# f4exb/sdrdaemon

Hardware: AMD Instinct MI355X
Metric: IQ Msamples/s through decim+FEC-encode pipe; bit-exact vs CPU ref (higher is better)
Workload: dtype int32

## Files before the change

sdrdaemon_amd/csrc/decim_body.h:

```cpp
#pragma once
#include "sdrhip_internal.h"

namespace sdrhip {
namespace {

constexpr int NT = 256;
constexpr int P0 = DECIM_PASS;
constexpr int FULL = 512;
constexpr int HE = 32;

typedef short short2_t __attribute__((ext_vector_type(2)));
typedef int int2_t __attribute__((ext_vector_type(2)));
typedef int int4_t __attribute__((ext_vector_type(4)));
typedef unsigned uint4_t __attribute__((ext_vector_type(4)));

constexpr int C64[16] = {-7, 11, -20, 32, -49, 71, -101, 140, -190, 256, -345, 469, -656, 978, -1698, 5201};
__host__ __device__ constexpr int H32(int i) { return i < 16 ? C64[i] : C64[31 - i]; }
__host__ __device__ constexpr unsigned pack_taps(int lo, int hi) { return ((unsigned)lo & 0xffffu) | ((unsigned)hi << 16); }

constexpr int PK0_DW = 16 + 512 + 16;
constexpr int I0_DW = 32 + 1024;
constexpr int SN_DW = 32 + FULL;

template <int NS_, bool PK_> struct Geo {
    static constexpr int NS = NS_;
    static constexpr bool PK = PK_;
    static constexpr int stride(int s) { return s == 0 ? (PK ? PK0_DW : I0_DW) : SN_DW; }
    static constexpr int base(int s) { return s == 0 ? 0 : base(s - 1) + 4 * stride(s - 1); }
    static constexpr int ldsDw = base(NS);
    static constexpr int plane(int s, int parity, int comp) { return base(s) + (parity * 2 + comp) * stride(s); }
};

__device__ __forceinline__ int dot2(unsigned a, unsigned taps, int acc)
{
    return __builtin_amdgcn_sdot2(__builtin_bit_cast(short2_t, a), __builtin_bit_cast(short2_t, taps), acc, false);
}

__device__ __forceinline__ int dot2_link(unsigned a, unsigned taps, int acc) { return dot2(a, taps, acc); }

__device__ __forceinline__ int dot2_init(unsigned a, unsigned taps, int c)
{
    int d;
    asm("v_dot2_i32_i16 %0, %1, %2, %3" : "=v"(d) : "v"(a), "s"(taps), "v"(c));
    return d;
}

__device__ __forceinline__ int mad24(int a, int tap, int acc)
{
    int d;
    asm("v_mad_i32_i24 %0, %1, %2, %3" : "=v"(d) : "v"(a), "s"(tap), "v"(acc));
    return d;
}

struct OutCtx {
    unsigned *out;
    size_t out_pos;
    bool store;
    int norm, trunk;
    int frame_mode, frame_blocks;
    uint64_t frame_sample_base;
};

__device__ __forceinline__ unsigned final_pack(int i, int q, int norm, int trunk)
{
    int a = (int)((unsigned)i << norm) >> trunk;
    int b = (int)((unsigned)q << norm) >> trunk;
    return ((unsigned)a & 0xffffu) | ((unsigned)b << 16);
}

__device__ __forceinline__ void store_one(const OutCtx &oc, size_t k, unsigned v)
{
    if (!oc.frame_mode) {
        oc.out[k] = v;
    } else {
        uint64_t g = oc.frame_sample_base + k;
        uint64_t f = g / 16129u;
        unsigned w = (unsigned)(g - f * 16129u);
        unsigned b = w / 127u, i = w - b * 127u;
        oc.out[((size_t)f * oc.frame_blocks + 1 + b) * 128u + 1 + i] = v;
    }
}

struct NoTaps { static constexpr bool ON = false; };
struct StageTaps {
    static constexpr bool ON = true;
    const DecimTapArgs &t;
    int stream;
    size_t pos[6];
};

template <class G, int S, class TAPS = NoTaps>
__device__ __forceinline__ void run_stage(int *lds, int tid, int valid, int fill_next, int bias, const OutCtx &oc, TAPS *taps = nullptr)
{
    constexpr bool PK = G::PK && S == 0;
    constexpr bool LAST = (S == G::NS - 1);
    constexpr int R = (S == 0) ? 8 : 4;
    const int j = tid >> 1, comp = tid & 1;
    const int k0 = j * R;
    if (k0 >= valid) return;
    const int *pe = lds + G::plane(S, 0, 0) + comp * G::stride(S);
    const int *po = lds + G::plane(S, 1, 0) + comp * G::stride(S);
    int res[R];
    if constexpr (PK) {
        constexpr int WO = (R + 32) / 2, WE = R / 2 + 4;
        unsigned wo[WO], we[WE];
#pragma unroll
        for (int d = 0; d < WO; d += 4) {
            uint4_t v = *reinterpret_cast<const uint4_t *>(po + k0 / 2 + d);
            wo[d] = v.x; wo[d + 1] = v.y; wo[d + 2] = v.z; wo[d + 3] = v.w;
        }
#pragma unroll
        for (int d = 0; d < WE; d += 4) {
            uint4_t v = *reinterpret_cast<const uint4_t *>(pe + k0 / 2 + 8 + d);
            we[d] = v.x; we[d + 1] = v.y; we[d + 2] = v.z; we[d + 3] = v.w;
        }
        const int bias13 = bias << 13;
        int acc[R];
#pragma unroll
        for (int r = 0; r < R; ++r)
            acc[r] = (r & 1) ? dot2_init(we[(r + 1) / 2], pack_taps(8192, 0), bias13) : dot2_init(we[r / 2], pack_taps(0, 8192), bias13);
#pragma unroll
        for (int t = 0; t < 17; ++t) {
#pragma unroll
            for (int r = 0; r < R; ++r) {
                if (r & 1) {
                    if (t < 16) acc[r] = dot2_link(wo[(r + 1) / 2 + t], pack_taps(H32(31 - 2 * t), H32(30 - 2 * t)), acc[r]);
                } else {
                    const unsigned taps = t == 0 ? pack_taps(0, H32(31)) : (t == 16 ? pack_taps(H32(0), 0) : pack_taps(H32(32 - 2 * t), H32(31 - 2 * t)));
                    acc[r] = dot2_link(wo[r / 2 + t], taps, acc[r]);
                }
            }
        }
#pragma unroll
        for (int r = 0; r < R; ++r) res[r] = acc[r] >> 13;
    } else {
        int wo[R + 32], we[R + 4];
#pragma unroll
        for (int x = 0; x < R + 32; x += 4) {
            int4_t v = *reinterpret_cast<const int4_t *>(po + k0 + x);
            wo[x] = v.x; wo[x + 1] = v.y; wo[x + 2] = v.z; wo[x + 3] = v.w;
        }
#pragma unroll
        for (int x = 0; x < R + 4; x += 4) {
            int4_t v = *reinterpret_cast<const int4_t *>(pe + k0 + 16 + x);
            we[x] = v.x; we[x + 1] = v.y; we[x + 2] = v.z; we[x + 3] = v.w;
        }
        int acc[R];
#pragma unroll
        for (int r = 0; r < R; ++r) acc[r] = (int)((unsigned)(we[r + 1] + bias) << 13);
#pragma unroll
        for (int i = 0; i < 16; ++i) {
#pragma unroll
            for (int r = 0; r < R; ++r) acc[r] = mad24(wo[r + 32 - i] + wo[r + 1 + i], C64[i], acc[r]);
        }
#pragma unroll
        for (int r = 0; r < R; ++r) res[r] = acc[r] >> 13;
    }

    if constexpr (LAST) {
        unsigned o[R];
#pragma unroll
        for (int r = 0; r < R; ++r) {
            int other = __builtin_amdgcn_update_dpp(0, res[r], 0xB1 , 0xf, 0xf, true);
            o[r] = final_pack(res[r], other, oc.norm, oc.trunk);
        }
        if (comp != 0 || !oc.store) return;
        const size_t k = oc.out_pos + k0;
        if (!oc.frame_mode && k0 + R <= valid) {
#pragma unroll
            for (int r = 0; r < R; r += 4) *reinterpret_cast<uint4_t *>(oc.out + k + r) = (uint4_t){o[r], o[r + 1], o[r + 2], o[r + 3]};
        } else if (!oc.frame_mode) {
#pragma unroll
            for (int r = 0; r < R; ++r)
                if (k0 + r < valid) oc.out[k + r] = o[r];
        } else {
            const uint64_t g = oc.frame_sample_base + k;
            const uint64_t f = g / 16129u;
            const unsigned w = (unsigned)(g - f * 16129u);
            unsigned b = w / 127u, i = w - b * 127u;
            size_t dw = ((size_t)f * oc.frame_blocks + 1 + b) * 128u + 1 + i;
#pragma unroll
            for (int r = 0; r < R; ++r) {
                if (k0 + r < valid) oc.out[dw] = o[r];
                ++i; ++dw;
                if (i == 127u) {
                    i = 0; ++b; dw += 1;
                    if (b == 127u) { b = 0; dw += ((size_t)oc.frame_blocks - 127u) * 128u; }
                }
            }
        }
    } else {
        int *ne = lds + G::plane(S + 1, 0, 0) + comp * G::stride(S + 1) + HE + fill_next + k0 / 2;
        int *no = lds + G::plane(S + 1, 1, 0) + comp * G::stride(S + 1) + HE + fill_next + k0 / 2;
        if constexpr (R == 8) {
            *reinterpret_cast<int4_t *>(ne) = (int4_t){res[0], res[2], res[4], res[6]};
            *reinterpret_cast<int4_t *>(no) = (int4_t){res[1], res[3], res[5], res[7]};
        } else {
            *reinterpret_cast<int2_t *>(ne) = (int2_t){res[0], res[2]};
            *reinterpret_cast<int2_t *>(no) = (int2_t){res[1], res[3]};
        }
        if constexpr (TAPS::ON) {
            if (oc.store && (taps->t.mask & (2u << S))) {
                const int norm = taps->t.norm[S + 1], trunk = taps->t.trunk[S + 1];
                unsigned o[R];
#pragma unroll
                for (int r = 0; r < R; ++r) {
                    int other = __builtin_amdgcn_update_dpp(0, res[r], 0xB1 , 0xf, 0xf, true);
                    o[r] = final_pack(res[r], other, norm, trunk);
                }
                if (comp == 0) {
                    unsigned *out = reinterpret_cast<unsigned *>(taps->t.out[S + 1]) + (size_t)taps->stream * taps->t.stride[S + 1] + taps->pos[S] + k0;
                    if (k0 + R <= valid) {
#pragma unroll
                        for (int r = 0; r < R; r += 4) *reinterpret_cast<uint4_t *>(out + r) = (uint4_t){o[r], o[r + 1], o[r + 2], o[r + 3]};
                    } else {
#pragma unroll
                        for (int r = 0; r < R; ++r)
                            if (k0 + r < valid) out[r] = o[r];
                    }
                }
            }
        }
    }
}

template <class G, int S> __device__ __forceinline__ void slide(int *lds, int tid, int consumed)
{
    if (tid >= 128) return;
    const int p = tid >> 5, e = tid & 31;
    int *pl = lds + G::base(S) + p * G::stride(S);
    if constexpr (G::PK && S == 0) {
        short *ps = reinterpret_cast<short *>(pl);
        const short v = ps[e + consumed];
        ps[e] = v;
    } else {
        const int v = pl[e + consumed];
        pl[e] = v;
    }
}

template <class G, int S> __device__ __forceinline__ void hist_put(int *lds, int p, int e, int v)
{
    int *pl = lds + G::base(S) + p * G::stride(S);
    if constexpr (G::PK && S == 0) reinterpret_cast<short *>(pl)[e] = (short)v;
    else pl[e] = v;
}
template <class G, int S> __device__ __forceinline__ int hist_get(const int *lds, int p, int e)
{
    const int *pl = lds + G::base(S) + p * G::stride(S);
    if constexpr (G::PK && S == 0) return reinterpret_cast<const short *>(pl)[e];
    else return pl[e];
}

template <class G, int S = 0> __device__ __forceinline__ void state_load(int *lds, int tid, const int32_t *st, bool zero)
{
    if (tid < 128) {
        const int sp = tid >> 5, e = tid & 31;
        const int kp = (sp & 1) * 2 + (sp >> 1);
        hist_put<G, S>(lds, kp, e, zero ? 0 : st[S * 4 * DEC_HIST + sp * DEC_HIST + e]);
    }
    if constexpr (S + 1 < G::NS) state_load<G, S + 1>(lds, tid, st, zero);
}
template <class G, int S = 0> __device__ __forceinline__ void state_store(const int *lds, int tid, int32_t *st)
{
    if (tid < 128) {
        const int sp = tid >> 5, e = tid & 31;
        const int kp = (sp & 1) * 2 + (sp >> 1);
        st[S * 4 * DEC_HIST + sp * DEC_HIST + e] = hist_get<G, S>(lds, kp, e);
    }
    if constexpr (S + 1 < G::NS) state_store<G, S + 1>(lds, tid, st);
}

template <class G, int S, class TAPS = NoTaps>
__device__ __forceinline__ void later_stages(int *lds, int tid, int (&fill)[6], int consumed_prev, bool flush, int bias, OutCtx &oc, TAPS *taps = nullptr)
{
    if constexpr (S < G::NS) {
        slide<G, S - 1>(lds, tid, consumed_prev);
        fill[S] += consumed_prev / 2;
        const int have = fill[S];
        const bool run = have > 0 && (have >= FULL || flush);
        if (run) {
            run_stage<G, S, TAPS>(lds, tid, have, fill[S + 1 < 6 ? S + 1 : 5], bias, oc, taps);
            if (S == G::NS - 1 && oc.store) oc.out_pos += have;
            if constexpr (TAPS::ON && S < G::NS - 1) {
                if (oc.store) taps->pos[S] += have;
            }
            fill[S] = 0;
        }
        __syncthreads();
        if (run) later_stages<G, S + 1, TAPS>(lds, tid, fill, have, flush, bias, oc, taps);
    } else {
        slide<G, G::NS - 1>(lds, tid, consumed_prev);
        __syncthreads();
    }
}

template <int L, int FC, bool PACK16, bool TAB = true, class TAPS = NoTaps>
__device__ __forceinline__ void decim_piece(const DecimArgs &a, int *lds, int stream, size_t seg_start, size_t seg_end, bool from_state,
                                            bool store_state, int meta_id, int meta_n, TAPS *taps = nullptr)
{
    constexpr bool CEN = (FC == 2);
    constexpr int NS = CEN ? L : L - 2;
    constexpr int RAWSH = CEN ? 0 : 2;
    constexpr int PRAW = P0 << RAWSH;
    constexpr int NLD = PRAW / 4 / NT;
    constexpr int WRAW = 64 << L;
    using G = Geo<NS, PACK16>;
    const int tid = threadIdx.x;
    const unsigned *in = reinterpret_cast<const unsigned *>(a.in) + (size_t)stream * a.in_stride;

    const int32_t *stc = a.state_cur + (size_t)stream * DEC_STATE_WORDS;
    state_load<G>(lds, tid, stc, !from_state);

    OutCtx oc;
    oc.norm = a.norm; oc.trunk = a.trunk;
    oc.frame_mode = a.frame_mode; oc.frame_blocks = a.frame_blocks; oc.frame_sample_base = a.frame_sample_base;
    oc.out = reinterpret_cast<unsigned *>(a.out) + (size_t)stream * a.out_stride;
    oc.out_pos = seg_start >> L;
    if constexpr (TAPS::ON) {
        static_assert(CEN, "taps: centred cascades only");
#pragma unroll
        for (int k = 0; k < 6; ++k) taps->pos[k] = seg_start >> (k + 1);
    }

    if (a.frame_mode) {
        unsigned base[6], rate;
        stream_meta_base(a.meta_w, a.meta_rate, TAB ? a.meta_tab : nullptr, stream, base, rate);
        for (int fi = meta_id + tid * meta_n; fi < a.meta_count; fi += NT * meta_n) {
            unsigned w[6];
            frame_meta_words_thread(base, a.meta_idx0, rate, fi, w);
            unsigned *fr = oc.out + (size_t)(a.meta_first + fi) * a.frame_blocks * 128u;
            fr[0] = (a.meta_frame_count0 + (unsigned)fi) & 0xffffu;
#pragma unroll
            for (int k = 0; k < 6; ++k) fr[1 + k] = w[k];
        }
        if (tid < 128) {
            for (int fi = meta_id; fi < a.meta_count; fi += meta_n) {
                unsigned *fr = oc.out + (size_t)(a.meta_first + fi) * a.frame_blocks * 128u;
                const unsigned fidx = (a.meta_frame_count0 + (unsigned)fi) & 0xffffu;
                if (tid >= 7) fr[tid] = 0u;
                if (tid >= 1) fr[(size_t)tid * 128] = fidx | ((unsigned)tid << 16);
            }
        }
    }

    int fill[6] = {0, 0, 0, 0, 0, 0};
    bool warm = !from_state;
    size_t pos = warm ? seg_start - WRAW : 0;
    size_t region_end = warm ? seg_start : seg_end;

    uint4_t ld[NLD];
    auto issue = [&](size_t p, size_t rend) {
        const unsigned *src = in + p;
        const size_t left = rend - p;
        if (left >= (size_t)PRAW) {
#pragma unroll
            for (int n = 0; n < NLD; ++n) ld[n] = SDRHIP_STREAM_LOAD(reinterpret_cast<const uint4_t *>(src + 4 * (tid + n * NT)));
            return;
        }
        const unsigned rem = (unsigned)left;
#pragma unroll
        for (int n = 0; n < NLD; ++n) {
            const unsigned q = (unsigned)(tid + n * NT);
            uint4_t v = (uint4_t){0u, 0u, 0u, 0u};
            if (4 * q + 3 < rem) {
                v = SDRHIP_STREAM_LOAD(reinterpret_cast<const uint4_t *>(src + 4 * q));
            } else if (4 * q < rem) {
                v.x = src[4 * q];
                if (4 * q + 1 < rem) v.y = src[4 * q + 1];
                if (4 * q + 2 < rem) v.z = src[4 * q + 2];
            }
            ld[n] = v;
        }
    };
    issue(pos, region_end);
    __syncthreads();

    while (true) {
        const size_t left = region_end - pos;
        const int cnt_raw = left < (size_t)PRAW ? (int)left : PRAW;
        const int cnt0 = cnt_raw >> RAWSH;
#pragma unroll
        for (int n = 0; n < NLD; ++n) {
            const int q = tid + n * NT;
            const uint4_t v = ld[n];
            if constexpr (CEN && PACK16) {
                lds[G::plane(0, 0, 0) + 16 + q] = (int)__builtin_amdgcn_perm(v.z, v.x, 0x05040100u);
                lds[G::plane(0, 0, 1) + 16 + q] = (int)__builtin_amdgcn_perm(v.z, v.x, 0x07060302u);
                lds[G::plane(0, 1, 0) + 16 + q] = (int)__builtin_amdgcn_perm(v.w, v.y, 0x05040100u);
                lds[G::plane(0, 1, 1) + 16 + q] = (int)__builtin_amdgcn_perm(v.w, v.y, 0x07060302u);
            } else if constexpr (CEN) {
                *reinterpret_cast<int2_t *>(&lds[G::plane(0, 0, 0) + HE + 2 * q]) = (int2_t){(int)(short)(v.x & 0xffff), (int)(short)(v.z & 0xffff)};
                *reinterpret_cast<int2_t *>(&lds[G::plane(0, 0, 1) + HE + 2 * q]) = (int2_t){(int)v.x >> 16, (int)v.z >> 16};
                *reinterpret_cast<int2_t *>(&lds[G::plane(0, 1, 0) + HE + 2 * q]) = (int2_t){(int)(short)(v.y & 0xffff), (int)(short)(v.w & 0xffff)};
                *reinterpret_cast<int2_t *>(&lds[G::plane(0, 1, 1) + HE + 2 * q]) = (int2_t){(int)v.y >> 16, (int)v.w >> 16};
            } else {
                const int I0 = (short)(v.x & 0xffff), Q0 = (int)v.x >> 16, I1 = (short)(v.y & 0xffff), Q1 = (int)v.y >> 16;
                const int I2 = (short)(v.z & 0xffff), Q2 = (int)v.z >> 16, I3 = (short)(v.w & 0xffff), Q3 = (int)v.w >> 16;
                int x, y;
                if constexpr (FC == 0) {
                    x = I0 - Q1 + Q3 - I2; y = Q0 - Q2 + I1 - I3;
                } else {
                    x = Q0 - I1 - Q2 + I3; y = -I0 - Q1 + I2 + Q3;
                }
                lds[G::plane(0, q & 1, 0) + HE + (q >> 1)] = x;
                lds[G::plane(0, q & 1, 1) + HE + (q >> 1)] = y;
            }
        }
        const size_t next_pos = pos + cnt_raw;
        const bool flush = next_pos >= region_end;
        bool more = !flush;
        size_t n_pos = next_pos, n_end = region_end;
        if (flush && warm && seg_start < seg_end) { more = true; n_pos = seg_start; n_end = seg_end; }
        if (more) issue(n_pos, n_end);
        __syncthreads();

        oc.store = !warm;
        const int valid0 = cnt0 >> 1;
        run_stage<G, 0, TAPS>(lds, tid, valid0, fill[1], a.bias, oc, taps);
        if (NS == 1 && oc.store) oc.out_pos += valid0;
        if constexpr (TAPS::ON && NS > 1) {
            if (oc.store) taps->pos[0] += valid0;
        }
        __syncthreads();
        later_stages<G, 1, TAPS>(lds, tid, fill, valid0, flush, a.bias, oc, taps);

        if (!more) break;
        if (flush) { warm = false; region_end = seg_end; }
        pos = n_pos;
    }

    if (store_state) {
        int32_t *stn = a.state_next + (size_t)stream * DEC_STATE_WORDS;
        state_store<G>(lds, tid, stn);
        for (int i = NS * 4 * DEC_HIST + tid; i < DEC_STAGES * 4 * DEC_HIST; i += NT) stn[i] = stc[i];
    }
}


template <int L, int FC, bool PACK16> struct DecimLds {
    static constexpr int NS = (FC == 2) ? L : L - 2;
    static constexpr int dwords = Geo<NS, PACK16>::ldsDw;
    static_assert(dwords * 4 <= 64 * 1024, "LDS budget");
};

__device__ __forceinline__ void decim_simple_row(int log2decim, int fcpos, const int16_t *in, size_t in_stride, int16_t *out,
                                                 size_t out_stride, size_t n_in, int norm, int trunk, int stream)
{
    const unsigned *src = reinterpret_cast<const unsigned *>(in) + (size_t)stream * in_stride;
    unsigned *dst = reinterpret_cast<unsigned *>(out) + (size_t)stream * out_stride;
    const size_t g = (size_t)blockIdx.x * blockDim.x + threadIdx.x;
    if (log2decim == 0) {
        for (size_t i = g; i < n_in; i += (size_t)gridDim.x * blockDim.x) {
            unsigned v = SDRHIP_STREAM_LOAD(src + i);
            int a = (short)(v & 0xffff), b = (int)v >> 16;
            dst[i] = (((unsigned)a << norm) & 0xffffu) | (((unsigned)b << norm) << 16);
        }
        return;
    }
    const size_t n_resize = n_in >> log2decim;
    const size_t ngroups = n_in / 4;
    for (size_t q = g; q < (n_in + 3) / 4; q += (size_t)gridDim.x * blockDim.x) {
        if (q >= ngroups) {
            if (log2decim == 1 && 2 * q < n_resize) dst[2 * q] = 0;
            continue;
        }
        const unsigned v0 = SDRHIP_STREAM_LOAD(src + 4 * q), v1 = SDRHIP_STREAM_LOAD(src + 4 * q + 1), v2 = SDRHIP_STREAM_LOAD(src + 4 * q + 2), v3 = SDRHIP_STREAM_LOAD(src + 4 * q + 3);
        const int I0 = (short)(v0 & 0xffff), Q0 = (int)v0 >> 16, I1 = (short)(v1 & 0xffff), Q1 = (int)v1 >> 16;
        const int I2 = (short)(v2 & 0xffff), Q2 = (int)v2 >> 16, I3 = (short)(v3 & 0xffff), Q3 = (int)v3 >> 16;
        if (log2decim == 1) {
            int xa, ya, xb, yb;
            if (fcpos == 0) { xa = I0 - Q1; ya = Q0 + I1; xb = Q3 - I2; yb = -Q2 - I3; }
            else { xa = Q0 - I1; ya = -I0 - Q1; xb = I3 - Q2; yb = I2 + Q3; }
            dst[2 * q] = final_pack(xa, ya, norm, trunk);
            dst[2 * q + 1] = final_pack(xb, yb, norm, trunk);
        } else {
            int x, y;
            if (fcpos == 0) { x = I0 - Q1 + Q3 - I2; y = Q0 - Q2 + I1 - I3; }
            else { x = Q0 - I1 - Q2 + I3; y = -I0 - Q1 + I2 + Q3; }
            dst[q] = final_pack(x, y, norm, trunk);
        }
    }
}

}
}
```

sdrdaemon_amd/csrc/decim_mfma.hip:

```cpp
#include "decim_body.h"

#include <type_traits>
#include <utility>

#ifndef MF_WAVES
#define MF_WAVES 2
#endif
#ifndef MF_DMA_BURST
#define MF_DMA_BURST 1
#endif

namespace sdrhip {
namespace {

__host__ __device__ constexpr int mf_entry(int kq, int t) { return 8 * (t >> 1) + 2 * kq + (t & 1); }

struct MfATab {
    unsigned w[2][4][64][4];
};

constexpr MfATab mf_make_atab()
{
    MfATab T{};
    for (int m = 0; m < 2; ++m)
// ... 173 lines not shown
            oc.p += oc.store ? 16 : 0;
        }
    }
}

struct MfFront {
    unsigned sel_own, sel_oth, sel_lo, sel_hi;
    unsigned ev_lo, ev_hi;
};
template <int NS, int I> __device__ __forceinline__ void mf_front(MfState<NS> &st, const MfConst &k, MfFront &f, const uint4_t r)
{
    constexpr int i = I;
    const unsigned ao = perm(r.w, r.y, f.sel_own), ae = perm(r.z, r.x, f.sel_own);
    const unsigned xo = perm(r.w, r.y, f.sel_oth), xe = perm(r.z, r.x, f.sel_oth);
    const unsigned yo = (unsigned)__builtin_amdgcn_update_dpp(0, (int)xo, 0xB1 , 0xf, 0xf, true);
    const unsigned ye = (unsigned)__builtin_amdgcn_update_dpp(0, (int)xe, 0xB1, 0xf, 0xf, true);
    st.O[0][0][i & 3] = (int)(perm(ao, yo, f.sel_lo) ^ 0x80808080u);
    st.O[0][1][i & 3] = (int)perm(ao, yo, f.sel_hi);
    const unsigned cur_lo = perm(ae, ye, f.sel_lo) ^ 0x80808080u, cur_hi = perm(ae, ye, f.sel_hi);
    st.O[0][0][(i + 1) & 3] = (int)perm(cur_lo, f.ev_lo, k.selA);
    st.O[0][1][(i + 1) & 3] = (int)perm(cur_hi, f.ev_hi, k.selA);
    f.ev_lo = cur_lo; f.ev_hi = cur_hi;
}

template <int NS, int I> __device__ __forceinline__ void mf_front2(MfState<NS> &st, const MfConst &k, MfFront &f, const uint4_t rA, const uint4_t rB)
{
    constexpr int i = I;
    const unsigned aoA = perm(rA.w, rA.y, f.sel_own), aoB = perm(rB.w, rB.y, f.sel_own);
    const unsigned aeA = perm(rA.z, rA.x, f.sel_own), aeB = perm(rB.z, rB.x, f.sel_own);
    st.O[0][0][i & 3] = (int)(perm(aoA, aoB, 0x01000504u) ^ 0x80808080u);
    st.O[0][1][i & 3] = (int)perm(aoA, aoB, 0x03020706u);
    const unsigned cur_lo = perm(aeA, aeB, 0x01000504u) ^ 0x80808080u, cur_hi = perm(aeA, aeB, 0x03020706u);
    st.O[0][0][(i + 1) & 3] = (int)perm(cur_lo, f.ev_lo, k.selA);
    st.O[0][1][(i + 1) & 3] = (int)perm(cur_hi, f.ev_hi, k.selA);
    f.ev_lo = cur_lo; f.ev_hi = cur_hi;
}

constexpr int MF_GROUP_BYTES = 9216;
constexpr int mf_wave_ring(int ng) { return ng * MF_GROUP_BYTES; }
static_assert(MF_HEAD_MIN % P0 == 0 && MF_TAIL_SEG % P0 == 0, "K1m's head and tail pieces are whole passes of the VALU code");
__host__ __device__ constexpr int mf_block_units(int p) { return 72 * p + 2 * (p >> 2); }

template <int D> __device__ __forceinline__ void mf_dma_issue(unsigned slot, unsigned voff, unsigned long long span_base)
{
    constexpr int off = 16 * mf_block_units(D);
    asm volatile("s_add_u32 m0, %1, %2\n\ts_nop 0\n\tglobal_load_lds_dwordx4 %0, %3 nt" ::"v"(voff), "s"(slot), "n"(off), "s"(span_base) : "memory", "scc");
}
template <int N> __device__ __forceinline__ void mf_wait_vm()
{
    static_assert(N == 0 || N == 7 || N == 8 || N == 15 || N == 16, "vmcnt immediates of the ring");
    if constexpr (N == 0) asm volatile("s_waitcnt vmcnt(0)" ::: "memory");
    if constexpr (N == 7) asm volatile("s_waitcnt vmcnt(7)" ::: "memory");
    if constexpr (N == 8) asm volatile("s_waitcnt vmcnt(8)" ::: "memory");
    if constexpr (N == 15) asm volatile("s_waitcnt vmcnt(15)" ::: "memory");
    if constexpr (N == 16) asm volatile("s_waitcnt vmcnt(16)" ::: "memory");
}

#ifdef MF_STAMPS
__device__ unsigned long long g_mf_stamps[4096 * 10];
__device__ __forceinline__ void mf_stamp(int gw, int k)
{
    if ((threadIdx.x & 63) == 0 && gw < 4096) {
        unsigned long long t;
        asm volatile("s_memrealtime %0\n\ts_waitcnt lgkmcnt(0)" : "=s"(t)::"memory");
        g_mf_stamps[gw * 10 + k] = t;
        if (k == 0) {
            unsigned hw, xcc;
            asm volatile("s_getreg_b32 %0, hwreg(HW_REG_HW_ID)" : "=s"(hw));
            asm volatile("s_getreg_b32 %0, hwreg(HW_REG_XCC_ID)" : "=s"(xcc));
            g_mf_stamps[gw * 10 + 8] = ((unsigned long long)(xcc & 0xfu) << 32) | hw;
        }
    }
}
#define MF_STAMP(gw, k) mf_stamp(gw, k)
#else
#define MF_STAMP(gw, k) do { } while (0)
#endif

template <int NS, int NG, class OC>
__device__ __forceinline__ void mf_loop_dma(const DecimArgs &a, MfState<NS> &st, const MfConst &k, OC &oc, MfFront &fr, unsigned lds_addr,
                                            const char *wbase, size_t S, int nper, int WP, int lane, int p, int comp, int q, int gw)
{
    constexpr int P = mf_period<NS>();
    static_assert(P == 32, "four groups of 8 steps per period");
    static_assert(NG == 2 || NG == 3 || NG == 4, "ring depth");
    constexpr int LA = NG - 1;
    const int wv = __builtin_amdgcn_readfirstlane((int)(threadIdx.x >> 6));
    const unsigned ring = (unsigned)__builtin_amdgcn_readfirstlane((int)(lds_addr + (unsigned)wv * (unsigned)mf_wave_ring(NG)));
    unsigned long long sb[8];
#pragma unroll
    for (int d = 0; d < 8; ++d) {
        const unsigned long long v = (unsigned long long)(wbase + (size_t)d * S * 4);
        sb[d] = ((unsigned long long)(unsigned)__builtin_amdgcn_readfirstlane((int)(v >> 32)) << 32) | (unsigned)__builtin_amdgcn_readfirstlane((int)v);
    }
    unsigned rs[NG];
    const __attribute__((address_space(3))) char *lr[NG];
#pragma unroll
    for (int j = 0; j < NG; ++j) {
        rs[j] = ring + (unsigned)(j * MF_GROUP_BYTES);
        lr[j] = (const __attribute__((address_space(3))) char *)(size_t)(rs[j] + 16u * (unsigned)(mf_block_units(0) + 72 * p + 2 * (p >> 2) + 4 * comp + q));
    }
    unsigned voff[4];
    const unsigned vmax = 16u * (unsigned)lane + 1024u * (unsigned)(4 * nper - 1);
#pragma unroll
    for (int g = 0; g < 4; ++g) voff[g] = min(16u * (unsigned)lane + 1024u * (unsigned)(g + LA), vmax);
    {
        unsigned v0 = 16u * (unsigned)lane;
        mf_static_for<8 * LA>([&](auto ic) {
            constexpr int i = decltype(ic)::value;
            mf_dma_issue<i % 8>(rs[i / 8], v0 + 1024u * (unsigned)(i / 8), sb[i % 8]);
        });
    }
    MF_STAMP(gw, 1);
    mf_wait_vm<8 * (LA - 1)>();
    uint4_t r = *reinterpret_cast<const __attribute__((address_space(3))) uint4_t *>(lr[0]);
    MF_STAMP(gw, 2);
    for (int per = 0; per < nper; ++per) {
#ifdef MF_STAMPS
        if (per == 1) MF_STAMP(gw, 3);
        if (per == nper / 4) MF_STAMP(gw, 4);
        if (per == nper / 2) MF_STAMP(gw, 5);
        if (per == 3 * nper / 4) MF_STAMP(gw, 6);
#endif
        oc.store = per >= WP;
        mf_static_for<P>([&](auto ic) {
            constexpr int i = decltype(ic)::value;
            constexpr int i1 = i + 1;
            constexpr int B = NG == 2 ? 8 : MF_DMA_BURST;
            if constexpr (i1 % 8 == 0) mf_wait_vm<(B == 1 ? 8 * (LA - 2) + 7 : 8 * (LA - 1))>();
            const uint4_t rn = *reinterpret_cast<const __attribute__((address_space(3))) uint4_t *>(lr[(i1 / 8) % NG] + 128 * (i1 % 8));
            constexpr int g = i / 8, d = i % 8;
            if constexpr (d < 8 / B) {
                mf_static_for<B>([&](auto bc) {
                    constexpr int sp = B * d + decltype(bc)::value;
                    mf_dma_issue<sp>(rs[(g + LA) % NG], voff[g], sb[sp]);
                });
                if constexpr (d == 8 / B - 1) voff[g] = min(voff[g] + 4096u, vmax);
            }
            mf_front<NS, i>(st, k, fr, r);
            mf_stage<NS, 0, i>(st, k, oc, comp);
            r = rn;
        });
        if constexpr (4 % NG != 0) {
            const unsigned t = rs[0];
            const __attribute__((address_space(3))) char *u = lr[0];
#pragma unroll
            for (int j = 0; j + 1 < NG; ++j) { rs[j] = rs[j + 1]; lr[j] = lr[j + 1]; }
            rs[NG - 1] = t; lr[NG - 1] = u;
        }
    }
    mf_wait_vm<0>();
}

template <int NS, int NG = 0, bool FR = false> __device__ __forceinline__ void mf_wave(const DecimArgs &a, int gw, unsigned lds_addr)
{
    if (a.mf_prio) __builtin_amdgcn_s_setprio(3);
    constexpr int L = NS;
    constexpr int P = mf_period<NS>();
#ifndef MF_DEPTH
#define MF_DEPTH 8
#endif
#ifndef MF_BURST
#define MF_BURST 1
#endif
    constexpr int D = MF_DEPTH < P ? MF_DEPTH : P / 2;
    constexpr size_t W = (size_t)64 << L;
    constexpr int WP = (int)(W / (32 * (size_t)P));
    static_assert(P % D == 0, "prefetch ring");
    static_assert((size_t)D * 32 <= MF_READ_AHEAD, "the planner leaves the register ring's read-ahead behind a wave's last span (decim_plan.h)");
    const int lane = threadIdx.x & 63;
    const int n = lane & 15, q = lane >> 4, comp = n & 1, p = n >> 1;
    const int stream = gw / a.mf_wps, ws = gw - stream * a.mf_wps;
    const size_t S = a.mf_span;
    const size_t wave_start = a.mf_head + (size_t)ws * 8 * S;
    const char *wbase = reinterpret_cast<const char *>(a.in) + ((size_t)stream * a.in_stride + wave_start - W) * 4;
    const unsigned loff = (unsigned)((size_t)p * S * 4) + 16u * (unsigned)q + 64u * (unsigned)comp;
    const int T = (int)((W + S) / 32);
    const int nper = T / P;

    MfConst k;
#pragma unroll
    for (int m = 0; m < 2; ++m)
#pragma unroll
        for (int ph = 0; ph < 4; ++ph) k.A[m][ph] = *reinterpret_cast<const int4_t *>(&mf_atab.w[m][ph][lane][0]);
    const unsigned b13 = (unsigned)a.bias << 13;
    const unsigned gain = (unsigned)mf_tap_sum() + 8192u;
    {
        const int c = (int)(128u * gain + b13);
        k.c0 = (int4_t){c, c, c, c};
    }
    k.cinN = (int)((unsigned)MF_LIMB_BIAS * gain + b13);
    k.selA = q == 0 ? 0x03020104u : 0x03020100u;
    k.selB = q == 0 ? 0x03020106u : 0x03020100u;

    MfOut<FR> oc;
    oc.store = 0;
    oc.dump = a.mf_dump + 4 * lane;
    oc.norm = a.norm; oc.trunk = a.trunk;
    oc.sel_pack = comp ? 0x01000504u : 0x05040100u;
    {
        const size_t first = ((wave_start + (size_t)p * S) >> L) + 4u * (unsigned)q;
        if constexpr (FR) {
            unsigned *obase = reinterpret_cast<unsigned *>(a.out) + (size_t)stream * a.out_stride;
            oc.rsrc = __builtin_amdgcn_make_buffer_rsrc(obase, 0, 0x3fffffff, 0x00020000);
            const unsigned long long g = a.frame_sample_base + first;
            const unsigned long long f = g / 16129u;
            const unsigned w = (unsigned)(g - f * 16129u);
            oc.b = w / 127u; oc.c = w - oc.b * 127u;
            oc.off = 4u * (unsigned)(((size_t)f * (size_t)a.frame_blocks + 1u + oc.b) * 128u + 1u + oc.c + 2u * (unsigned)comp);
            oc.t0 = 127u - 2u * (unsigned)comp; oc.t1 = 126u - 2u * (unsigned)comp;
            oc.gap = 4u * ((unsigned)a.frame_blocks * 128u - 16255u);
            oc.p = nullptr;
        } else {
            unsigned *obase = reinterpret_cast<unsigned *>(a.out) + (size_t)stream * a.out_stride;
            oc.p = obase + first + 2 * comp;
            oc.off = oc.c = oc.b = oc.t0 = oc.t1 = oc.gap = 0u;
        }
    }

    MfState<NS> st;
#pragma unroll
    for (int s = 0; s < NS; ++s) {
#pragma unroll
        for (int b = 0; b < 3; ++b) st.O[s][b] = (int4_t){0, 0, 0, 0};
        st.pend[s][0] = st.pend[s][1] = 0u;
        st.evp[s][0] = st.evp[s][1] = 0u;
    }

    MfFront fr;
    fr.sel_own = comp ? 0x07030602u : 0x05010400u;
    fr.sel_oth = comp ? 0x05010400u : 0x07030602u;
    fr.sel_lo = comp ? 0x05040100u : 0x01000504u; fr.sel_hi = comp ? 0x07060302u : 0x03020706u;
    fr.ev_lo = 0u; fr.ev_hi = 0u;
    if constexpr (NG != 0 && mf_dma_applies(NS)) {
        mf_loop_dma<NS, NG>(a, st, k, oc, fr, lds_addr, wbase, S, nper, WP, lane, p, comp, q, gw);
        return;
    }
    uint4_t ld[D];
    const char *src = wbase + loff;
#define MF_LDSTRIDE 128
#pragma unroll
    for (int d = 0; d < D; ++d) ld[d] = SDRHIP_STREAM_LOAD(reinterpret_cast<const uint4_t *>(src + MF_LDSTRIDE * d));

    for (int per = 0; per < nper; ++per) {
        oc.store = per >= WP;
        mf_static_for<P>([&](auto ic) {
            constexpr int i = decltype(ic)::value;
            constexpr int slot = i % D;
            const uint4_t r = ld[slot];
            ld[slot] = SDRHIP_STREAM_LOAD(reinterpret_cast<const uint4_t *>(src + MF_LDSTRIDE * (i + D)));
            mf_front<NS, i>(st, k, fr, r);
            mf_stage<NS, 0, i>(st, k, oc, comp);
        });
        src += MF_LDSTRIDE * P;
    }
}

__host__ __device__ constexpr int mf_block_threads(int) { return NT; }

template <int L, bool PACK16, int NG, bool FR> __global__ __launch_bounds__(mf_block_threads(L), mf_dma_applies(L) && NG != 2 ? 1 : MF_WAVES) void decim_mfma_kernel(DecimArgs a)
{
    constexpr int LDSDW = mf_dma_applies(L) && mf_wave_ring(NG) > DecimLds<L, 2, PACK16>::dwords ? mf_wave_ring(NG) : DecimLds<L, 2, PACK16>::dwords;
    __shared__ __attribute__((aligned(16))) int lds[LDSDW];
    const int nmf = (a.nstreams * a.mf_wps + 3) / 4;
    const int bx = blockIdx.x;
    if (bx >= nmf) {
        const int nitems = a.nstreams * a.mf_npieces, j = bx - nmf, nearly = a.mf_piece_early * a.mf_piece_share;
        const int nmine = j < a.mf_piece_early ? a.mf_piece_share : 1;
        for (int k = 0; k < nmine; ++k) {
            const int lx = j < a.mf_piece_early ? j + k * a.mf_piece_early : nearly + (j - a.mf_piece_early);
            if (lx >= nitems || (j < a.mf_piece_early && lx >= nearly)) break;
            const int stream = lx / a.mf_npieces, piece = lx - stream * a.mf_npieces;
            if (piece == 0) {
                decim_piece<L, 2, PACK16>(a, lds, stream, 0, a.mf_head, true, false, piece, a.mf_npieces);
            } else {
                const size_t s0 = a.mf_tail_start + (size_t)(piece - 1) * a.mf_tail_seg;
                size_t s1 = s0 + a.mf_tail_seg;
                if (s1 > a.n_used || piece == a.mf_npieces - 1) s1 = a.n_used;
                decim_piece<L, 2, PACK16>(a, lds, stream, s0, s1, false, piece == a.mf_npieces - 1, piece, a.mf_npieces);
            }
            __syncthreads();
        }
        return;
    }
    const int gw = __builtin_amdgcn_readfirstlane(bx * 4 + (int)(threadIdx.x >> 6));
    if (gw >= a.nstreams * a.mf_wps) return;
    MF_STAMP(gw, 0);
    mf_wave<L, NG, FR>(a, gw, (unsigned)(size_t)(__attribute__((address_space(3))) char *)lds);
    MF_STAMP(gw, 7);
}
__device__ __forceinline__ int mf_ragged_find(const RaggedRow *rows, int nstreams, int x, bool waves)
{
    int lo = 0, hi = nstreams - 1;
    while (lo < hi) {
        const int mid = (lo + hi + 1) >> 1;
        if ((waves ? rows[mid].mf_w0 : rows[mid].mf_p0) <= x) lo = mid;
        else hi = mid - 1;
    }
    return __builtin_amdgcn_readfirstlane(lo);
}
__device__ __forceinline__ DecimArgs mf_ragged_args(const DecimArgs &a, const RaggedRow &r)
{
    DecimArgs b = a;
    b.n_used = (size_t)r.n_used;
    b.mf_wps = r.mf_wps;
    const unsigned sh = (unsigned)__builtin_amdgcn_readfirstlane((int)r.shifts);
    b.norm = (int)(sh & 0xffu); b.trunk = (int)(sh >> 8);
    if (a.frame_mode) {
        b.out = reinterpret_cast<int16_t *>(reinterpret_cast<unsigned *>(a.out) + r.out_off);
        b.frame_sample_base = r.frame_sample_base;
        b.meta_first = r.meta_first; b.meta_count = r.meta_count; b.meta_frame_count0 = r.frame_count0;
        b.meta_w[3] = r.tv_sec; b.meta_w[4] = r.tv_usec;
        b.meta_idx0 = r.meta_idx0;
    }
    return b;
}

template <int L, bool PACK16, int NG, bool FR> __global__ __launch_bounds__(mf_block_threads(L), mf_dma_applies(L) && NG != 2 ? 1 : MF_WAVES) void decim_mfma_ragged_kernel(DecimArgs a, const RaggedRow *rows)
{
    constexpr int LDSDW = mf_dma_applies(L) && mf_wave_ring(NG) > DecimLds<L, 2, PACK16>::dwords ? mf_wave_ring(NG) : DecimLds<L, 2, PACK16>::dwords;
    __shared__ __attribute__((aligned(16))) int lds[LDSDW];
    const int nmf = (a.mf_wps + 3) / 4;
    const int bx = blockIdx.x;
    if (bx >= nmf) {
        const int nitems = a.mf_npieces, j = bx - nmf, nearly = a.mf_piece_early * a.mf_piece_share;
        const int nmine = j < a.mf_piece_early ? a.mf_piece_share : 1;
        for (int k = 0; k < nmine; ++k) {
            const int lx = j < a.mf_piece_early ? j + k * a.mf_piece_early : nearly + (j - a.mf_piece_early);
            if (lx >= nitems || (j < a.mf_piece_early && lx >= nearly)) break;
            const int stream = mf_ragged_find(rows, a.nstreams, lx, false);
            const RaggedRow &r = rows[stream];
            const DecimArgs b = mf_ragged_args(a, r);
            const int piece = lx - r.mf_p0;
            const size_t n_used = (size_t)r.n_used;
            if (piece == 0) {
                decim_piece<L, 2, PACK16, false>(b, lds, stream, 0, (size_t)r.mf_head, true, r.mf_np == 1, piece, r.mf_np);
            } else {
                const size_t s0 = (size_t)r.mf_tail_start + (size_t)(piece - 1) * a.mf_tail_seg;
                size_t s1 = s0 + a.mf_tail_seg;
                if (s1 > n_used || piece == r.mf_np - 1) s1 = n_used;
                decim_piece<L, 2, PACK16, false>(b, lds, stream, s0, s1, false, piece == r.mf_np - 1, piece, r.mf_np);
            }
            __syncthreads();
        }
        return;
    }
    const int gw = __builtin_amdgcn_readfirstlane(bx * 4 + (int)(threadIdx.x >> 6));
    if (gw >= a.mf_wps) return;
    const int stream = mf_ragged_find(rows, a.nstreams, gw, true);
    const RaggedRow &r = rows[stream];
    const DecimArgs b = mf_ragged_args(a, r);
    mf_wave<L, NG, FR>(b, stream * r.mf_wps + (gw - r.mf_w0), (unsigned)(size_t)(__attribute__((address_space(3))) char *)lds);
}

#ifdef MF_STAMPS
}
extern "C" int sdrhip_debug_mf_stamps(unsigned long long *dst) { return (int)hipMemcpyFromSymbol(dst, HIP_SYMBOL(g_mf_stamps), sizeof(g_mf_stamps)); }
namespace {
#endif

#include "gf_encode128_body.h"
#ifndef MF_FUSED_WPE
#define MF_FUSED_WPE 3
#endif
struct FusedRoles {
    unsigned *tab;
    unsigned tag;
};

template <int L, bool PACK16> __global__ __launch_bounds__(NT, MF_FUSED_WPE) void rx_fused_kernel(DecimArgs a, Enc128Args e, FusedRoles fr)
{
    constexpr int LDSDW = ENC128_LDS_BYTES / 4 > DecimLds<L, 2, PACK16>::dwords ? ENC128_LDS_BYTES / 4 : DecimLds<L, 2, PACK16>::dwords;
    __shared__ __attribute__((aligned(16))) int lds[LDSDW];
    __shared__ int s_unit;
    const int nmf = (a.nstreams * a.mf_wps + 3) / 4;
    const int npiece = a.nstreams * a.mf_npieces;
    const int nenc = 2 * e.nlist;
    if (threadIdx.x == 0) {
        unsigned hw, xcc;
        asm volatile("s_getreg_b32 %0, hwreg(HW_REG_HW_ID)" : "=s"(hw));
        asm volatile("s_getreg_b32 %0, hwreg(HW_REG_XCC_ID)" : "=s"(xcc));
        const unsigned key = ((xcc & 0xfu) << 8) | ((hw >> 8) & 0xffu);
        unsigned *cnt = fr.tab + 4096 + 4 * (fr.tag & 1u);
        if (blockIdx.x == 0) { unsigned *nxt = fr.tab + 4096 + 4 * ((fr.tag + 1u) & 1u); nxt[0] = 0u; nxt[1] = 0u; nxt[2] = 0u; }
        const bool first = atomicMax(fr.tab + key, fr.tag) < fr.tag;
        int unit = -1;
        if (first) { const unsigned u = atomicAdd(cnt + 0, 1u); if (u < (unsigned)nmf) unit = (int)u; }
        if (unit < 0) { const unsigned u = atomicAdd(cnt + 1, 1u); if (u < (unsigned)npiece) unit = nmf + (int)u; }
        if (unit < 0) { const unsigned u = atomicAdd(cnt + 2, 1u); if (u < (unsigned)nenc) unit = nmf + npiece + (int)u; }
        if (unit < 0) { const unsigned u = atomicAdd(cnt + 0, 1u); if (u < (unsigned)nmf) unit = (int)u; }
        s_unit = unit;
    }
    __syncthreads();
    const int bx = s_unit;
    if (bx < 0) return;
    const int ndec = nmf + npiece;
    if (bx >= ndec) {
        gf_encode128_wg(e, bx - ndec, reinterpret_cast<unsigned char *>(lds));
        return;
    }
    if (bx >= nmf) {
        const int lx = bx - nmf;
        const int stream = lx / a.mf_npieces, piece = lx - stream * a.mf_npieces;
        if (piece == 0) {
            decim_piece<L, 2, PACK16>(a, lds, stream, 0, a.mf_head, true, false, piece, a.mf_npieces);
        } else {
            const size_t s0 = a.mf_tail_start + (size_t)(piece - 1) * a.mf_tail_seg;
            size_t s1 = s0 + a.mf_tail_seg;
            if (s1 > a.n_used || piece == a.mf_npieces - 1) s1 = a.n_used;
            decim_piece<L, 2, PACK16>(a, lds, stream, s0, s1, false, piece == a.mf_npieces - 1, piece, a.mf_npieces);
        }
        return;
    }
    const int gw = __builtin_amdgcn_readfirstlane(bx * 4 + (int)(threadIdx.x >> 6));
    if (gw >= a.nstreams * a.mf_wps) return;
    mf_wave<L, 0>(a, gw, 0u);
}

template <int L> hipError_t launch_fused(bool pack16, const DecimArgs &a, const Enc128Args &e, unsigned *roles, unsigned tag, hipStream_t stream)
{
    const int ndec = (a.nstreams * a.mf_wps + 3) / 4 + a.nstreams * a.mf_npieces;
    const dim3 grid(ndec + 2 * e.nlist), block(NT);
    FusedRoles fr;
    fr.tab = roles; fr.tag = tag;
    if (pack16) hipLaunchKernelGGL((rx_fused_kernel<L, true>), grid, block, 0, stream, a, e, fr);
    else hipLaunchKernelGGL((rx_fused_kernel<L, false>), grid, block, 0, stream, a, e, fr);
    return hipGetLastError();
}

template <int L, int NG, bool FR> void launch_mf2(bool pack16, const DecimArgs &a, dim3 grid, dim3 block, hipStream_t stream)
{
    if (pack16) hipLaunchKernelGGL((decim_mfma_kernel<L, true, NG, FR>), grid, block, 0, stream, a);
    else hipLaunchKernelGGL((decim_mfma_kernel<L, false, NG, FR>), grid, block, 0, stream, a);
}

template <int L> hipError_t launch_mf(bool pack16, const DecimArgs &a, hipStream_t stream)
{
    const int nleg = a.mf_piece_wgs > 0 ? a.mf_piece_wgs : a.nstreams * a.mf_npieces;
    const int nmf = (a.nstreams * a.mf_wps + 3) / 4;
    const dim3 grid(nleg + nmf), block(mf_block_threads(L));
    if constexpr (mf_dma_applies(L)) {
// ... 76 lines not shown
```

sdrdaemon_amd/csrc/rx_frame_area.h:

```cpp
#pragma once
#include <cstddef>
#include <cstdint>
#include <vector>

namespace sdrhip {
constexpr uint64_t RX_FRAME_SAMPLES = 127 * 127;
constexpr size_t RX_NO_LATE = ~(size_t)0;

struct RxAdvance {
    size_t done;
    uint64_t rest;
    int first_new;
    int started;
    uint64_t idx0;
    unsigned frame_count0;
};

struct RxAreaPlan {
    size_t new_cap = 0;
    bool keep_old = false;
    std::vector<uint8_t> to_slot0;
    bool moves() const
    {
        for (size_t s = 0; s < to_slot0.size(); ++s)
            if (to_slot0[s]) return true;
        return false;
    }
};

class RxFrameArea {
public:
    void init(size_t nstreams)
    {
        cap_ = 0;
        base_.assign(nstreams, 0); pending_.assign(nstreams, 0); open_.assign(nstreams, 0); count_.assign(nstreams, 0);
    }
    size_t streams() const { return base_.size(); }
    size_t cap() const { return cap_; }
    size_t slot(size_t s) const { return base_[s]; }
    const size_t *slots() const { return base_.data(); }
    uint64_t pending(size_t s) const { return pending_[s]; }
    bool open(size_t s) const { return open_[s] != 0; }
    uint16_t count(size_t s) const { return count_[s]; }
    size_t index(size_t s, size_t f = 0) const { return s * cap_ + base_[s] + f; }

    bool aligned() const
    {
        for (size_t s = 1; s < base_.size(); ++s)
            if (base_[s] != base_[0] || pending_[s] != pending_[0] || open_[s] != open_[0] || count_[s] != count_[0]) return false;
        return true;
    }

    RxAdvance advance(size_t s, size_t n_dec) const
    {
        RxAdvance a;
        const uint64_t total = pending_[s] + n_dec;
        a.done = (size_t)(total / RX_FRAME_SAMPLES);
        a.rest = total - (uint64_t)a.done * RX_FRAME_SAMPLES;
        a.first_new = open_[s] ? 1 : 0;
        a.started = (int)(a.done + (a.rest > 0 ? 1 : 0)) - a.first_new;
        a.idx0 = a.first_new ? RX_FRAME_SAMPLES - pending_[s] : 0;
        a.frame_count0 = (unsigned)count_[s] + (unsigned)a.first_new;
        return a;
    }

    RxAreaPlan plan(const size_t *done, size_t late_slot0, size_t window_multiple) const
    {
        RxAreaPlan p;
        const size_t S = base_.size();
        size_t need_max = 0;
        for (size_t s = 0; s < S; ++s) need_max = done[s] + 1 > need_max ? done[s] + 1 : need_max;
        bool hits_late = false;
        p.to_slot0.assign(S, 0);
        if (need_max > cap_) p.new_cap = window_multiple * need_max;
        else
            for (size_t s = 0; s < S; ++s) {
                if (base_[s] + done[s] + 1 <= cap_) continue;
                p.to_slot0[s] = 1;
                hits_late = hits_late || (late_slot0 != RX_NO_LATE && done[s] + 1 > late_slot0);
            }
        if (hits_late) p.new_cap = cap_;
        if (p.new_cap) {
            p.to_slot0.assign(S, 1);
            p.keep_old = late_slot0 != RX_NO_LATE;
        }
        return p;
    }
    RxAreaPlan replan() const
    {
        RxAreaPlan p;
        p.new_cap = cap_;
        p.to_slot0.assign(base_.size(), cap_ ? 1 : 0);
        return p;
    }
    void moved(const RxAreaPlan &p)
    {
        if (p.new_cap) cap_ = p.new_cap;
        for (size_t s = 0; s < base_.size(); ++s)
            if (p.to_slot0[s]) base_[s] = 0;
    }
    void commit(const size_t *done, const uint64_t *rest)
    {
        for (size_t s = 0; s < base_.size(); ++s) {
            base_[s] += done[s];
            pending_[s] = rest[s];
            open_[s] = rest[s] > 0 ? 1 : 0;
            count_[s] = (uint16_t)(count_[s] + done[s]);
        }
    }

    void reset(const uint8_t *mask)
    {
        for (size_t s = 0; s < base_.size(); ++s) {
            if (mask && !mask[s]) continue;
            pending_[s] = 0; open_[s] = 0; count_[s] = 0;
            if (!mask) base_[s] = 0;
        }
    }
    static bool importable(uint64_t pending, uint32_t open, uint32_t count)
    {
        return open <= 1 && pending < RX_FRAME_SAMPLES && (open || !pending) && count <= 0xffffu;
    }
    void import_stream(size_t s, uint64_t pending, uint32_t open, uint32_t count)
    {
        pending_[s] = pending; open_[s] = (uint8_t)open; count_[s] = (uint16_t)count;
    }

private:
    size_t cap_ = 0;
    std::vector<size_t> base_;
    std::vector<uint64_t> pending_;
    std::vector<uint8_t> open_;
    std::vector<uint16_t> count_;
};

class RxView {
public:
    const uint8_t *base() const { return base_; }
    size_t stride() const { return stride_; }
    size_t first(size_t s) const { return first_[s]; }
    size_t frames(size_t s) const { return frames_[s]; }
    void init(size_t nstreams) { set(nullptr, 0, nstreams, 0, 0); }
    void clear() { base_ = nullptr; stride_ = 0; first_.assign(first_.size(), 0); frames_.assign(frames_.size(), 0); }
    bool uniform() const
    {
        for (size_t s = 1; s < first_.size(); ++s)
            if (first_[s] != first_[0] || frames_[s] != frames_[0]) return false;
        return true;
    }
    void set(const uint8_t *area, size_t stream_stride, size_t nstreams, size_t first_slot, size_t n)
    {
        base_ = area; stride_ = stream_stride; first_.assign(nstreams, first_slot); frames_.assign(nstreams, n);
    }
    void set_each(const uint8_t *area, size_t stream_stride, size_t nstreams, const size_t *first_slot, const size_t *n)
    {
        base_ = area; stride_ = stream_stride; first_.assign(first_slot, first_slot + nstreams); frames_.assign(n, n + nstreams);
    }
    size_t offset(size_t s, size_t frame_bytes) const { return s * stride_ + first_[s] * frame_bytes; }
    const uint8_t *window(size_t s, size_t frame_bytes) const { return base_ ? base_ + offset(s, frame_bytes) : nullptr; }

private:
    const uint8_t *base_ = nullptr;
    size_t stride_ = 0;
    std::vector<size_t> first_, frames_;
};
}
```

sdrdaemon_amd/csrc/sdrhip.cpp:

```cpp
#include "sdrhip_host.h"
#include "gf256.h"

#include <cstdarg>
#include <cstdio>
#include <cstdlib>
#include <cstring>
#include <new>
#include <string>
#include <vector>

using namespace sdrhip;

namespace {
thread_local std::string g_err;
}

namespace sdrhip {

int fail(int code, const char *fmt, ...)
{
    char buf[512];
    va_list ap;
    va_start(ap, fmt);
    vsnprintf(buf, sizeof(buf), fmt, ap);
    va_end(ap);
    g_err = buf;
    return code;
}

}

extern "C" const char *sdrhip_last_error(void) { return g_err.c_str(); }

extern "C" int sdrhip_device_count(void)
{
    int n = 0;
    if (hipGetDeviceCount(&n) != hipSuccess) return 0;
    return n;
}

namespace sdrhip {
static void ctx_free(sdrhip_ctx *c);
static void drop_kernel_events(sdrhip_ctx *c)
{
    (void)hipStreamSynchronize(c->stream);
    if (c->stream2) (void)hipStreamSynchronize(c->stream2);
    for (int k = 0; k < SDRHIP_KCLASSES; ++k) {
        for (auto &pr : c->kev[k]) { (void)hipEventDestroy(pr.first); (void)hipEventDestroy(pr.second); }
        c->kev[k].clear();
    }
}
}

extern "C" int sdrhip_ctx_create(int device, void *hip_stream, sdrhip_ctx **out)
{
    if (!out) return fail(SDRHIP_EINVAL, "ctx_create: out is NULL");
    *out = nullptr;
    int n = sdrhip_device_count();
    if (n <= 0) return fail(SDRHIP_EDEVICE, "no HIP device available (this library has no CPU fallback)");
    if (device < 0 || device >= n) return fail(SDRHIP_EINVAL, "device %d out of range (have %d)", device, n);
    HIP_TRY(hipSetDevice(device));
    sdrhip_ctx *c = new (std::nothrow) sdrhip_ctx();
    if (!c) return fail(SDRHIP_ENOMEM, "out of host memory");
    c->device = device;
    c->stream = static_cast<hipStream_t>(hip_stream);
    {
        hipDeviceProp_t prop;
        if (hipGetDeviceProperties(&prop, device) == hipSuccess && prop.multiProcessorCount > 0) c->n_cu = prop.multiProcessorCount;
        static const char *const keys[][2] = {{"SDRHIP_DECIM_PATH", "decim_path"}, {"SDRHIP_MFMA_SPAN", "mfma_span"}, {"SDRHIP_MFMA_MIN", "mfma_min"},
                                              {"SDRHIP_INTERP_PATH", "interp_path"}, {"SDRHIP_INTERP_SPAN", "interp_span"}, {"SDRHIP_RX_FUSED", "rx_fused"}, {"SDRHIP_RX_DIRECT", "rx_direct"},
                                              {"SDRHIP_DEC_PATH", "dec_path"}, {"SDRHIP_ENC_PATH", "enc_path"}, {"SDRHIP_ENC_MIN_ROWS", "enc_min_rows"}, {"SDRHIP_MFMA_RING", "mfma_ring"}, {"SDRHIP_TX_OVERLAP", "tx_overlap"}, {"SDRHIP_RX_WINDOW", "rx_window"}, {"SDRHIP_FEC_STAGGER", "fec_stagger"}, {"SDRHIP_FEC_STAGGER_MOD", "fec_stagger_mod"}, {"SDRHIP_DEC_PLAN", "dec_plan"}, {"SDRHIP_TX_GATHER", "tx_gather"}, {"SDRHIP_ENC_UNITS", "enc_units"}, {"SDRHIP_ENC_FORM", "enc_form"}};
        for (size_t i = 0; i < sizeof(keys) / sizeof(keys[0]); ++i)
            if (const char *v = getenv(keys[i][0])) (void)sdrhip_ctx_set_option(c, keys[i][1], v);
    }
    std::vector<uint8_t> tab(256 * 32);
    gf_build_tables(tab.data());
    if (hipMalloc(reinterpret_cast<void **>(&c->gf_tab), tab.size()) != hipSuccess) { c->gf_tab = nullptr; ctx_free(c); return fail(SDRHIP_ENOMEM, "hipMalloc gf tables"); }
    if (hipMemcpy(c->gf_tab, tab.data(), tab.size(), hipMemcpyHostToDevice) != hipSuccess) { ctx_free(c); return fail(SDRHIP_EDEVICE, "upload gf tables"); }
    std::vector<uint8_t> em(128 * 128);
    cm256_encode_matrix(128, 128, em.data());
    if (hipMalloc(reinterpret_cast<void **>(&c->enc_matrix), em.size()) != hipSuccess ||
        hipMemcpy(c->enc_matrix, em.data(), em.size(), hipMemcpyHostToDevice) != hipSuccess) { ctx_free(c); return fail(SDRHIP_ENOMEM, "upload encode matrix"); }
    std::vector<uint8_t> kl(8 * 81 * 32);
    cm256_karatsuba_leaf_tables(kl.data());
    if (hipMalloc(reinterpret_cast<void **>(&c->enc_leaves), kl.size()) != hipSuccess ||
        hipMemcpy(c->enc_leaves, kl.data(), kl.size(), hipMemcpyHostToDevice) != hipSuccess) { ctx_free(c); return fail(SDRHIP_ENOMEM, "upload encoder constants"); }
    {
        std::vector<uint8_t> ft((size_t)CM256_FFT_TABLES * 32);
        cm256_fft_tables(ft.data());
        if (hipMalloc(reinterpret_cast<void **>(&c->enc_fft), ft.size()) != hipSuccess ||
            hipMemcpy(c->enc_fft, ft.data(), ft.size(), hipMemcpyHostToDevice) != hipSuccess) { ctx_free(c); return fail(SDRHIP_ENOMEM, "upload encoder FFT constants"); }
    }
    {
        const GF256 &g = gf();
        uint8_t el[1024];
        memcpy(el, g.exp, 512);
        memcpy(el + 512, g.log, 512);
        if (hipMalloc(reinterpret_cast<void **>(&c->gf_explog), sizeof(el)) != hipSuccess ||
            hipMemcpy(c->gf_explog, el, sizeof(el), hipMemcpyHostToDevice) != hipSuccess) { ctx_free(c); return fail(SDRHIP_ENOMEM, "upload GF(256) exp/log tables"); }
    }
    if (hipMalloc(reinterpret_cast<void **>(&c->dec_stats), 64) != hipSuccess ||
        hipMemset(c->dec_stats, 0, 64) != hipSuccess) { ctx_free(c); return fail(SDRHIP_ENOMEM, "hipMalloc decoder counters"); }
    if (hipMalloc(reinterpret_cast<void **>(&c->decim_dump), 4096) != hipSuccess) { c->decim_dump = nullptr; ctx_free(c); return fail(SDRHIP_ENOMEM, "hipMalloc decimator scratch"); }
    if (hipMalloc(reinterpret_cast<void **>(&c->fused_roles), SDRHIP_FUSED_ROLE_WORDS * 4) != hipSuccess ||
        hipMemset(c->fused_roles, 0, SDRHIP_FUSED_ROLE_WORDS * 4) != hipSuccess) { ctx_free(c); return fail(SDRHIP_ENOMEM, "hipMalloc role table"); }
    if (hipEventCreate(&c->ev0) != hipSuccess || hipEventCreate(&c->ev1) != hipSuccess) { ctx_free(c); return fail(SDRHIP_EDEVICE, "hipEventCreate"); }
    *out = c;
    return SDRHIP_OK;
}

namespace sdrhip {
int ctx_stream2(sdrhip_ctx *c, hipStream_t *out)
{
    if (!c->stream2) {
        int lo = 0, hi = 0;
        if (hipDeviceGetStreamPriorityRange(&lo, &hi) != hipSuccess) lo = 0;
        if (hipStreamCreateWithPriority(&c->stream2, hipStreamNonBlocking, lo) != hipSuccess) {
            c->stream2 = nullptr;
            return fail(SDRHIP_EDEVICE, "hipStreamCreate (second stream)");
        }
    }
    *out = c->stream2;
    return SDRHIP_OK;
}
void ctx_retain(sdrhip_ctx *c) { c->refs.fetch_add(1); }
void ctx_release(sdrhip_ctx *c)
{
    if (c->refs.fetch_sub(1) == 1 && c->dying) ctx_free(c);
}
}

extern "C" void sdrhip_ctx_destroy(sdrhip_ctx *c)
{
    if (!c || c->dying.exchange(true)) return;
    if (c->refs.load() == 0) ctx_free(c);
}

extern "C" int sdrhip_ctx_set_option(sdrhip_ctx *c, const char *key, const char *value)
{
    if (!c || !key || !value) return fail(SDRHIP_EINVAL, "ctx_set_option: NULL argument");
    sdrhip::CtxLock lock_(c);
    const std::string k(key), v(value);
    char *end = nullptr;
    const unsigned long long num = strtoull(value, &end, 10);
    const bool isnum = *value && end && !*end;
    if (k == "decim_path") {
        if (v == "auto") c->opt.decim_path = DECIM_PATH_AUTO;
        else if (v == "valu") c->opt.decim_path = DECIM_PATH_VALU;
        else if (v == "mfma") c->opt.decim_path = DECIM_PATH_MFMA;
        else return fail(SDRHIP_EINVAL, "ctx_set_option: decim_path must be auto, valu or mfma");
    } else if (k == "interp_path") {
        if (v == "auto") c->opt.interp_wave = CtxOptions().interp_wave;
        else if (v == "valu") c->opt.interp_wave = 0;
        else if (v == "wave") c->opt.interp_wave = 1;
        else return fail(SDRHIP_EINVAL, "ctx_set_option: interp_path must be auto, valu or wave");
    } else if (k == "mfma_span" && isnum) c->opt.mfma_span = (size_t)num;
    else if (k == "mfma_min" && isnum) c->opt.mfma_min = (size_t)num;
    else if (k == "interp_span" && isnum) c->opt.interp_span = (size_t)num;
    else if (k == "rx_fused" && isnum && num <= 3) c->opt.rx_fused = (int)num;
    else if (k == "rx_fused" && v == "overlap") c->opt.rx_fused = 3;
    else if (k == "rx_direct" && isnum && num <= 1) c->opt.rx_direct = (int)num;
    else if (k == "rx_window" && isnum && num <= 8) c->opt.rx_window = (int)num;
    else if (k == "mfma_ring" && isnum && num >= 2 && num <= 4) c->opt.mfma_ring = (int)num;
    else if (k == "tx_overlap" && isnum && num <= 1) c->opt.tx_overlap = (int)num;
    else if (k == "fec_stagger" && isnum && num <= 64) c->opt.fec_stagger = (int)num;
    else if (k == "fec_stagger_mod" && isnum && num <= 116) c->opt.fec_stagger_mod = (int)num;
    else if (k == "tx_gather" && isnum && num <= 1) c->opt.tx_gather = (int)num;
    else if (k == "dec_plan") {
        if (v == "fused") c->opt.dec_fused_plan = 1;
        else if (v == "kernel") c->opt.dec_fused_plan = 0;
        else return fail(SDRHIP_EINVAL, "ctx_set_option: dec_plan must be fused or kernel");
    }
    else if (k == "enc_min_rows" && isnum && num >= 1 && num <= 32) c->opt.enc_min_rows = (int)num;
    else if (k == "enc_units" && (v == "frame" || v == "half")) c->opt.enc_half = v == "half";
    else if (k == "enc_form" && (v == "bitslice" || v == "table")) c->opt.enc_bitslice = v == "bitslice";
    else if (k == "enc_path") {
        if (v == "fft") c->opt.enc_fft = 1;
        else if (v == "karatsuba") c->opt.enc_fft = 0;
        else return fail(SDRHIP_EINVAL, "ctx_set_option: enc_path must be fft or karatsuba");
    } else if (k == "dec_path") {
        if (v == "syndrome") c->opt.dec_syndrome = 1;
        else if (v == "dense") c->opt.dec_syndrome = 0;
        else return fail(SDRHIP_EINVAL, "ctx_set_option: dec_path must be syndrome or dense");
    } else if (k == "dec_max_rows" && isnum && num >= 1 && num <= 128) { c->opt.dec_max_rows = (int)num; c->opt.dec_auto = 0; }
    else if (k == "dec_max_rows" && v == "auto") { c->opt.dec_max_rows = 128; c->opt.dec_auto = 1; }
    else if (k == "dec_strict" && isnum && num <= 1) c->opt.dec_strict = (int)num;
    else if (k == "ktime_stride" && isnum && num >= 1 && num <= 1024) { c->ktime_stride = (int)num; for (int i = 0; i < SDRHIP_KCLASSES; ++i) c->ktime_stride_cls[i] = 0; }
    else if (k == "ktime_stride_class") {
        int cls = -1, st = 0;
        if (sscanf(value, "%d:%d", &cls, &st) != 2 || cls < 0 || cls >= SDRHIP_KCLASSES || st < 1 || st > 1024) return fail(SDRHIP_EINVAL, "ctx_set_option: ktime_stride_class takes <class 0..4>:<stride 1..1024>");
        c->ktime_stride_cls[cls] = st;
    }
    else return fail(SDRHIP_EINVAL, "ctx_set_option: unknown key or malformed value: %s=%s", key, value);
    return SDRHIP_OK;
}

extern "C" int sdrhip_ctx_get_counter(sdrhip_ctx *c, const char *key, uint64_t *value)
{
    if (!c || !key || !value) return fail(SDRHIP_EINVAL, "ctx_get_counter: NULL argument");
    sdrhip::CtxLock lock_(c);
    if (std::string(key) == "h2d_bytes") { *value = c->h2d_bytes; return SDRHIP_OK; }
    if (std::string(key) == "d2h_bytes") { *value = c->d2h_bytes; return SDRHIP_OK; }
    const bool shadow = std::string(key) == "fecbuf_shadow_mismatch";
    const bool deferred = std::string(key) == "dec_deferred";
    if (std::string(key) != "dec_rows_exceeded" && !shadow && !deferred) return fail(SDRHIP_EINVAL, "ctx_get_counter: unknown key: %s", key);
    HIP_TRY(hipSetDevice(c->device));
    unsigned v = 0;
    HIP_TRY(link_copy(c, &v, c->dec_stats + (shadow ? DEC_STATS_SHADOW_MISMATCH : deferred ? DEC_STATS_DEFERRED : 0), sizeof(v), hipMemcpyDeviceToHost, c->stream));
    HIP_TRY(hipStreamSynchronize(c->stream));
    *value = v;
    return SDRHIP_OK;
}

int sdrhip::enc128_min_rows(const sdrhip_ctx *c) { return c->opt.enc_fft ? c->opt.enc_min_rows : ENC128_MIN_ROWS; }

static void sdrhip::ctx_free(sdrhip_ctx *c)
{
    (void)hipSetDevice(c->device);
    (void)hipStreamSynchronize(c->stream);
    drop_kernel_events(c);
    c->in.release(); c->out.release(); c->aux.release(); c->aux3.release();
    if (c->gf_tab) (void)hipFree(c->gf_tab);
    if (c->enc_matrix) (void)hipFree(c->enc_matrix);
    if (c->enc_leaves) (void)hipFree(c->enc_leaves);
    if (c->enc_fft) (void)hipFree(c->enc_fft);
    if (c->decim_dump) (void)hipFree(c->decim_dump);
    if (c->fused_roles) (void)hipFree(c->fused_roles);
    if (c->gf_explog) (void)hipFree(c->gf_explog);
    if (c->dec_stats) (void)hipFree(c->dec_stats);
    c->dec_plan.release();
    c->pin.release();
    c->zin.release(); c->zout.release();
    if (c->stream2) { (void)hipStreamSynchronize(c->stream2); (void)hipStreamDestroy(c->stream2); }
    if (c->ev0) (void)hipEventDestroy(c->ev0);
    if (c->ev1) (void)hipEventDestroy(c->ev1);
    delete c;
}

extern "C" int sdrhip_ctx_synchronize(sdrhip_ctx *c)
{
    if (!c) return fail(SDRHIP_EINVAL, "ctx is NULL");
    sdrhip::CtxLock lock_(c);
    HIP_TRY(hipStreamSynchronize(c->stream));
    if (c->stream2) HIP_TRY(hipStreamSynchronize(c->stream2));
    return SDRHIP_OK;
}

extern "C" int sdrhip_ctx_timing_begin(sdrhip_ctx *c)
{
    if (!c) return fail(SDRHIP_EINVAL, "ctx is NULL");
    HIP_TRY(hipEventRecord(c->ev0, c->stream));
    return SDRHIP_OK;
}

extern "C" int sdrhip_ctx_timing_end(sdrhip_ctx *c, float *ms)
{
    if (!c || !ms) return fail(SDRHIP_EINVAL, "ctx/ms is NULL");
    HIP_TRY(hipEventRecord(c->ev1, c->stream));
    HIP_TRY(hipEventSynchronize(c->ev1));
    HIP_TRY(hipEventElapsedTime(ms, c->ev0, c->ev1));
    return SDRHIP_OK;
}

extern "C" int sdrhip_ctx_kernel_timing(sdrhip_ctx *c, int enable)
{
    if (!c) return fail(SDRHIP_EINVAL, "ctx is NULL");
    sdrhip::CtxLock lock_(c);
    c->ktime_on = enable != 0;
    for (int i = 0; i < SDRHIP_KCLASSES; ++i) c->ktime_seen[i] = 0;
    if (!enable) drop_kernel_events(c);
    return SDRHIP_OK;
}

extern "C" int sdrhip_ctx_kernel_timing_read(sdrhip_ctx *c, int cls, double *total_ms, unsigned *launches)
{
    if (!c || cls < 0 || cls >= SDRHIP_KCLASSES || !total_ms || !launches) return fail(SDRHIP_EINVAL, "kernel_timing_read: bad argument");
    sdrhip::CtxLock lock_(c);
    HIP_TRY(hipStreamSynchronize(c->stream));
    if (c->stream2) HIP_TRY(hipStreamSynchronize(c->stream2));
    double sum = 0;
    unsigned n = 0;
    for (auto &pr : c->kev[cls]) {
        float ms = 0;
        if (hipEventElapsedTime(&ms, pr.first, pr.second) == hipSuccess) { sum += ms; ++n; }
        (void)hipEventDestroy(pr.first);
        (void)hipEventDestroy(pr.second);
    }
    c->kev[cls].clear();
    *total_ms = sum;
    *launches = n;
    return SDRHIP_OK;
}

namespace {
struct HostRange { const char *p; size_t n; };
std::mutex g_host_mtx;
std::vector<HostRange> g_host_ranges;
}
namespace sdrhip {
bool host_is_pinned(const void *p, size_t n)
{
    std::lock_guard<std::mutex> g(g_host_mtx);
    const char *c = static_cast<const char *>(p);
    for (const HostRange &r : g_host_ranges)
        if (c >= r.p && c + n <= r.p + r.n) return true;
    return false;
}
}

extern "C" void *sdrhip_host_alloc(sdrhip_ctx *c, size_t bytes)
{
    if (!c || bytes == 0) return nullptr;
    if (hipSetDevice(c->device) != hipSuccess) return nullptr;
    void *p = nullptr;
    if (hipHostMalloc(&p, bytes, hipHostMallocDefault) != hipSuccess) { (void)fail(SDRHIP_ENOMEM, "hipHostMalloc(%zu) failed", bytes); return nullptr; }
    std::lock_guard<std::mutex> g(g_host_mtx);
    g_host_ranges.push_back(HostRange{static_cast<const char *>(p), bytes});
    return p;
}

extern "C" void sdrhip_host_free(sdrhip_ctx *c, void *p)
{
    if (!p) return;
    (void)c;
    {
        std::lock_guard<std::mutex> g(g_host_mtx);
        for (size_t i = 0; i < g_host_ranges.size(); ++i)
            if (g_host_ranges[i].p == p) { g_host_ranges.erase(g_host_ranges.begin() + (long)i); break; }
    }
    (void)hipHostFree(p);
}
```

sdrdaemon_amd/csrc/sdrhip_decim.cpp:

```cpp
#include "sdrhip_host.h"

#include <cstring>
#include <new>
#include <vector>

using namespace sdrhip;

struct sdrhip_decimators {
    sdrhip::CtxRef ctx;
    int nstreams;
    int bias;
    sdrhip::DevBuf state[2];
    int cur;
    bool stage0_int16;
    sdrhip::DecimPlanInfo last;
    sdrhip::PinnedBuf rows_pin, stage_pin, out_pin;
    sdrhip::DevBuf rows_dev;
    sdrhip::StreamMask reset_mask;
    explicit sdrhip_decimators(sdrhip_ctx *c) : ctx(c) {}
};

extern "C" int sdrhip_decimators_last_plan(const sdrhip_decimators *d, sdrhip_decim_plan *out)
{
    if (!d || !out) return fail(SDRHIP_EINVAL, "decimators_last_plan: NULL argument");
    sdrhip::CtxLock lock_(d->ctx);
    out->path = d->last.path; out->wps = d->last.wps; out->npieces = d->last.npieces; out->nseg = d->last.nseg;
    out->span = d->last.span; out->head = d->last.head; out->tail_start = d->last.tail_start;
    return SDRHIP_OK;
}

extern "C" int sdrhip_decimators_create(sdrhip_ctx *ctx, int nstreams, int hb_variant, sdrhip_decimators **out)
{
    if (!ctx || !out || nstreams <= 0 || nstreams > 65535) return fail(SDRHIP_EINVAL, "decimators_create: bad argument");
    if (hb_variant != SDRHIP_HB_EO1 && hb_variant != SDRHIP_HB_DB) return fail(SDRHIP_EINVAL, "hb_variant must be SDRHIP_HB_EO1 or SDRHIP_HB_DB");
    HIP_TRY(hipSetDevice(ctx->device));
    sdrhip_decimators *d = new (std::nothrow) sdrhip_decimators(ctx);
    if (!d) return fail(SDRHIP_ENOMEM, "out of host memory");
    d->nstreams = nstreams; d->bias = hb_variant; d->cur = 0; d->stage0_int16 = true;
    size_t bytes = (size_t)nstreams * DEC_STATE_WORDS * sizeof(int32_t);
    if (d->state[0].alloc_exact(bytes) || d->state[1].alloc_exact(bytes)) {
        delete d;
        return fail(SDRHIP_ENOMEM, "hipMalloc decimator state");
    }
    *out = d;
    return sdrhip_decimators_reset(d);
}

extern "C" void sdrhip_decimators_destroy(sdrhip_decimators *d)
{
    if (!d) return;
    (void)hipSetDevice(d->ctx->device);
    (void)hipStreamSynchronize(d->ctx->stream);
    delete d;
}

extern "C" int sdrhip_decimators_reset(sdrhip_decimators *d)
{
    if (!d) return fail(SDRHIP_EINVAL, "decimators is NULL");
    sdrhip::CtxLock lock_(d->ctx);
    size_t bytes = (size_t)d->nstreams * DEC_STATE_WORDS * sizeof(int32_t);
    HIP_TRY(hipMemsetAsync(d->state[0].p, 0, bytes, d->ctx->stream));
    HIP_TRY(hipMemsetAsync(d->state[1].p, 0, bytes, d->ctx->stream));
    d->cur = 0;
    d->stage0_int16 = true;
    return SDRHIP_OK;
}

namespace sdrhip {
void decimators_reset_part(sdrhip_decimators *d, StreamResetArgs *a)
{
    a->rows[0] = d->state[0].as<int32_t>(); a->rows[1] = d->state[1].as<int32_t>();
    a->row_words = DEC_STATE_WORDS;
}
void decimators_reset_done(sdrhip_decimators *d, bool all)
{
    if (all) d->stage0_int16 = true;
}
int32_t *decimators_row(sdrhip_decimators *d, int s, int half) { return d->state[d->cur ^ (half & 1)].as<int32_t>() + (size_t)s * DEC_STATE_WORDS; }
bool decimators_stage0_int16(const sdrhip_decimators *d) { return d->stage0_int16; }
void decimators_clear_stage0_int16(sdrhip_decimators *d) { d->stage0_int16 = false; }
}

extern "C" int sdrhip_decimators_reset_streams(sdrhip_decimators *d, const uint8_t *mask)
{
    if (!d) return fail(SDRHIP_EINVAL, "decimators is NULL");
    sdrhip::CtxLock lock_(d->ctx);
    return stream_reset_bank(d->ctx, d->reset_mask, mask, d->nstreams,
                             [d](StreamResetArgs *a) { decimators_reset_part(d, a); },
                             [d](const uint8_t *m) { decimators_reset_done(d, m == nullptr); });
}

namespace {
void set_mf_args(DecimArgs &a, const MfPlan &p)
{
    a.mf_head = p.head; a.mf_span = p.span; a.mf_tail_start = p.tail_start; a.mf_tail_seg = p.tail_seg;
    a.mf_wps = p.wps; a.mf_npieces = p.npieces;
    a.mf_piece_wgs = p.piece_wgs; a.mf_piece_early = p.piece_early; a.mf_piece_share = p.piece_share;
}

struct DecimCall {
    const int16_t *in;
    size_t in_stride;
    int16_t *out;
    size_t out_stride;
    int frame_mode, frame_blocks;
    size_t n_raw, n_dec;
    size_t min_used;
};

template <class Simple, class Plan, class Launch>
int decimate_core(sdrhip_decimators *d, unsigned L, int fcpos, const DecimCall &k, Simple simple, Plan plan, Launch launch)
{
    sdrhip_ctx *c = d->ctx;
    d->last = DecimPlanInfo();
    if ((L == 0 ? k.n_raw : k.n_dec) == 0) return SDRHIP_OK;
    const bool cen = fcpos == SDRHIP_FC_CEN;
    if (L == 0 || (!cen && L <= 2)) {
        if (k.frame_mode) return fail(SDRHIP_EINVAL, L == 0 ? "internal: frame mode needs log2decim >= 1" : "internal: frame mode unsupported for filter-less decimation");
        hipError_t e = simple();
        if (e != hipSuccess) return fail(SDRHIP_EDEVICE, "decimate%u launch: %s", 1u << L, hipGetErrorString(e));
        return SDRHIP_OK;
    }

    DecimArgs a;
    memset(&a, 0, sizeof(a));
    a.in = k.in; a.out = k.out; a.in_stride = k.in_stride; a.out_stride = k.out_stride;
    a.state_cur = d->state[d->cur].as<int32_t>(); a.state_next = d->state[d->cur ^ 1].as<int32_t>();
    a.nstreams = d->nstreams;
    a.bias = d->bias;
    a.frame_mode = k.frame_mode; a.frame_blocks = k.frame_blocks;
    a.mf_dump = c->decim_dump;
    bool mfma = false;
    if (int rc = plan(a, &mfma)) return rc;
    const bool pack16 = cen && d->stage0_int16;
    hipError_t e;
    {
        KTimer kt(c, SDRHIP_K_DECIMATE);
        e = launch(a, pack16, mfma);
    }
    if (e != hipSuccess) return fail(SDRHIP_EDEVICE, "decimate launch: %s", hipGetErrorString(e));
    d->last.path = mfma ? DECIM_PATH_MFMA : DECIM_PATH_VALU;
    if (mfma) {
        d->last.span = a.mf_span; d->last.head = a.mf_head; d->last.tail_start = a.mf_tail_start;
        d->last.wps = a.mf_wps; d->last.npieces = a.mf_npieces;
    } else {
        d->last.nseg = a.nseg;
    }
    d->cur ^= 1;
    d->stage0_int16 = cen && (d->stage0_int16 || k.min_used >= (size_t)2 * DEC_HIST);
    return SDRHIP_OK;
}
}

namespace sdrhip {
int decimate_device(sdrhip_decimators *d, int log2decim, int fcpos, unsigned *sampleSize, const int16_t *in, size_t n_in,
                    size_t in_stride, int16_t *out, size_t out_stride, size_t *n_out, int frame_mode, int frame_blocks,
                    uint64_t frame_sample_base, const RxMeta *meta, const Enc128Args *fuse, bool *fused, bool coresident)
{
    if (fused) *fused = false;
    sdrhip_ctx *c = d->ctx;
    const int S = d->nstreams;
    const unsigned L = (unsigned)log2decim;
    const DecimShifts sh = decimated_shifts(L, *sampleSize);
    const size_t n_dec = n_in >> L;
    const size_t n_used = n_dec << L;
    *sampleSize = decimated_sample_size(L, *sampleSize);
    if (n_out) *n_out = n_dec;
    const DecimCall k = {in, in_stride, out, out_stride, frame_mode, frame_blocks, n_in, n_dec, n_used};
    return decimate_core(
        d, L, fcpos, k,
        [&]() { return launch_decimate_simple(log2decim, fcpos, in, in_stride, out, out_stride, n_in, S, (int)sh.norm, (int)sh.trunk, c->stream); },
        [&](DecimArgs &a, bool *mfma) -> int {
            a.n_used = n_used;
            a.norm = (int)sh.norm; a.trunk = (int)sh.trunk;
            a.frame_sample_base = frame_sample_base;
            if (meta) set_meta_args(a, *meta);
            plan_decimate(log2decim, fcpos, n_used, S, &a.nsub_per_seg, &a.nseg);
            const CtxOptions &env = c->opt;
            const bool mfma_frames = env.rx_direct && out_stride * 4 < 0x3fffffffu;
            a.mf_ring = coresident ? 3 : env.mfma_ring;
            a.mf_prio = coresident ? 1 : 0;
            MfPlan p;
            *mfma = (!frame_mode || mfma_frames) && mfma_admitted(env.decim_path, env.mfma_min, log2decim, n_used * (size_t)S) &&
                    plan_decimate_mfma(log2decim, fcpos, n_used, S, env.mfma_span, c->n_cu, a.mf_ring, &p);
            if (*mfma) set_mf_args(a, p);
            return SDRHIP_OK;
        },
        [&](const DecimArgs &a, bool pack16, bool mfma) -> hipError_t {
            if (!(mfma && fuse && L <= 4))
                return mfma ? launch_decimate_mfma(log2decim, pack16, a, c->stream) : launch_decimate(log2decim, fcpos, pack16, a, c->stream);
            hipError_t e;
            if (++c->fused_tag == 0xffffffffu) {
                (void)hipMemsetAsync(c->fused_roles, 0, SDRHIP_FUSED_ROLE_WORDS * 4, c->stream);
                c->fused_tag = 1;
            }
            if (c->opt.rx_fused == 2) {
                Enc128Args none = *fuse;
                none.nlist = 0;
                e = launch_rx_fused(log2decim, pack16, a, none, c->fused_roles, c->fused_tag, c->stream);
                if (e == hipSuccess) e = launch_gf_encode128(*fuse, c->stream);
            } else
                e = launch_rx_fused(log2decim, pack16, a, *fuse, c->fused_roles, c->fused_tag, c->stream);
            if (e != hipSuccess) {
                (void)hipMemsetAsync(c->fused_roles, 0, SDRHIP_FUSED_ROLE_WORDS * 4, c->stream);
                c->fused_tag = 0;
            }
            if (fused) *fused = true;
            return e;
        });
}

bool decimate_mfma_applies(const sdrhip_decimators *d, int log2decim, int fcpos, size_t n_in)
{
    const CtxOptions &env = d->ctx->opt;
    const size_t n_used = (n_in >> log2decim) << log2decim;
    MfPlan p;
    return mfma_admitted(env.decim_path, env.mfma_min, log2decim, n_used * (size_t)d->nstreams) &&
           plan_decimate_mfma(log2decim, fcpos, n_used, d->nstreams, env.mfma_span, d->ctx->n_cu, env.mfma_ring, &p);
}
}

extern "C" int sdrhip_decimate(sdrhip_decimators *d, int log2decim, int fcpos, unsigned *sampleSize, const int16_t *iq_in,
                               size_t n_in, size_t in_stride, int16_t *iq_out, size_t out_stride, size_t *n_out, int mem)
{
    if (!d || !sampleSize) return fail(SDRHIP_EINVAL, "decimate: NULL handle or sampleSize");
    sdrhip::CtxLock lock_(d->ctx);
    if (log2decim < 0 || log2decim > 6) return fail(SDRHIP_EINVAL, "Invalid log2 decimation factor");
    if (fcpos < SDRHIP_FC_INF || fcpos > SDRHIP_FC_CEN) return fail(SDRHIP_EINVAL, "Invalid Fc position index");
    if (*sampleSize < 1 || *sampleSize > 16) return fail(SDRHIP_EINVAL, "sampleSize must be 1..16");
    if (n_in && (!iq_in || (!iq_out && (n_in >> log2decim)))) return fail(SDRHIP_EINVAL, "decimate: NULL buffer");
    sdrhip_ctx *c = d->ctx;
    HIP_TRY(hipSetDevice(c->device));
    const int S = d->nstreams;
    const size_t n_res = n_in >> log2decim;
    if (S == 1) { in_stride = n_in; out_stride = n_res; }
    if (S > 1 && (in_stride < n_in || out_stride < n_res)) return fail(SDRHIP_EINVAL, "decimate: stride smaller than the per-stream length");

    if (mem == SDRHIP_MEM_DEVICE) {
        if (n_in && (!aligned16(iq_in) || !aligned16(iq_out) || (S > 1 && ((in_stride & 3) || (out_stride & 3)))))
            return fail(SDRHIP_EALIGN, "decimate: device pointers must be 16-byte aligned and strides multiples of 4 samples");
        return decimate_device(d, log2decim, fcpos, sampleSize, iq_in, n_in, in_stride, iq_out, out_stride, n_out, 0, 0, 0);
    }
    if (int e = check_mem(mem)) return e;

    const size_t dis = (n_in + 3) & ~(size_t)3, dos = (n_res + 3) & ~(size_t)3;
    if (n_in == 0)
        return decimate_device(d, log2decim, fcpos, sampleSize, nullptr, 0, 0, nullptr, 0, n_out, 0, 0, 0);
    int rc;
    if ((size_t)S * dis * 4 <= SDRHIP_ZEROCOPY_MAX) {
        if ((rc = c->zin.reserve((size_t)S * dis * 4 + 16))) return rc;
        if ((rc = c->zout.reserve((size_t)S * dos * 4 + 16))) return rc;
        for (int s = 0; s < S; ++s) memcpy(c->zin.as<int16_t>() + (size_t)s * dis * 2, iq_in + (size_t)s * in_stride * 2, n_in * 4);
        link_bytes(c, hipMemcpyHostToDevice, (size_t)S * n_in * 4);
        link_bytes(c, hipMemcpyDeviceToHost, (size_t)S * n_res * 4);
        rc = decimate_device(d, log2decim, fcpos, sampleSize, c->zin.as<int16_t>(), n_in, dis, c->zout.as<int16_t>(), dos, n_out, 0, 0, 0);
        if (rc) return rc;
        HIP_TRY(hipStreamSynchronize(c->stream));
        for (int s = 0; s < S && n_res; ++s) memcpy(iq_out + (size_t)s * out_stride * 2, c->zout.as<int16_t>() + (size_t)s * dos * 2, n_res * 4);
        return SDRHIP_OK;
    }
    if ((rc = c->in.reserve((size_t)S * dis * 4 + 16))) return rc;
    if ((rc = c->out.reserve((size_t)S * dos * 4 + 16))) return rc;
    HIP_TRY(link_copy2d(c, c->in.p, dis * 4, iq_in, in_stride * 4, n_in * 4, S, hipMemcpyHostToDevice, c->stream));
    rc = decimate_device(d, log2decim, fcpos, sampleSize, static_cast<const int16_t *>(c->in.p), n_in, dis,
                         static_cast<int16_t *>(c->out.p), dos, n_out, 0, 0, 0);
    if (rc) return rc;
    if (n_res) HIP_TRY(link_copy2d(c, iq_out, out_stride * 4, c->out.p, dos * 4, n_res * 4, S, hipMemcpyDeviceToHost, c->stream));
    HIP_TRY(hipStreamSynchronize(c->stream));
    return SDRHIP_OK;
}

namespace sdrhip {
int ragged_prepare(sdrhip_decimators *d, int log2decim, int fcpos, const size_t *n_in, RaggedRow *rows, const RaggedRow **rows_dev,
                   RaggedPlan *plan, PinnedBuf *pin)
{
    sdrhip_ctx *c = d->ctx;
    const int S = d->nstreams;
    size_t total = 0;
    for (int s = 0; s < S; ++s) {
        rows[s].n_raw = n_in[s];
        rows[s].n_dec = n_in[s] >> log2decim;
        rows[s].n_used = (uint64_t)(n_in[s] >> log2decim) << log2decim;
        total += (size_t)rows[s].n_used;
    }
    if (!plan_decimate_ragged(log2decim, fcpos, rows, S, total, &plan->nsub, &plan->grid)) return fail(SDRHIP_EINVAL, "ragged call: too many segments");
    const CtxOptions &env = c->opt;
    plan->ring = env.mfma_ring == 3 ? 3 : 4;
    plan->mfma = mfma_admitted(env.decim_path, env.mfma_min, log2decim, total) &&
                 plan_decimate_mfma_ragged(log2decim, fcpos, rows, S, env.mfma_span, c->n_cu, plan->ring, &plan->mf);
    const size_t bytes = (size_t)S * sizeof(RaggedRow);
    int rc;
    PinnedBuf &tab = pin ? *pin : d->rows_pin;
    if ((rc = tab.reserve(bytes))) return rc;
    if ((rc = d->rows_dev.reserve(bytes))) return rc;
    memcpy(tab.p, rows, bytes);
    HIP_TRY(hipMemcpyAsync(d->rows_dev.p, tab.p, bytes, hipMemcpyHostToDevice, c->stream));
    tab.mark(c->stream);
    *rows_dev = d->rows_dev.as<RaggedRow>();
    return SDRHIP_OK;
}

int ragged_reserve(sdrhip_decimators *d, PinnedBuf *pin)
{
    const size_t bytes = (size_t)d->nstreams * sizeof(RaggedRow);
    if (int rc = (pin ? *pin : d->rows_pin).reserve(bytes)) return rc;
    return d->rows_dev.reserve(bytes);
}

int decimate_ragged_device(sdrhip_decimators *d, int log2decim, int fcpos, unsigned *sampleSize, const int16_t *in, size_t in_stride,
                           int16_t *out, size_t out_stride, const RaggedRow *rows, const RaggedRow *rows_dev, const RaggedPlan &plan,
                           int frame_mode, int frame_blocks, const unsigned *meta_w, unsigned meta_rate)
{
    sdrhip_ctx *c = d->ctx;
    const int S = d->nstreams;
    const unsigned L = (unsigned)log2decim;
    size_t max_raw = 0, max_dec = 0, min_used = SIZE_MAX;
    for (int s = 0; s < S; ++s) {
        if (rows[s].n_raw > max_raw) max_raw = (size_t)rows[s].n_raw;
        if (rows[s].n_dec > max_dec) max_dec = (size_t)rows[s].n_dec;
        if (rows[s].n_used < min_used) min_used = (size_t)rows[s].n_used;
    }
    for (int s = 0; s < S; ++s) sampleSize[s] = decimated_sample_size(L, sampleSize[s]);
    const DecimCall k = {in, in_stride, out, out_stride, frame_mode, frame_blocks, max_raw, max_dec, min_used};
    return decimate_core(
        d, L, fcpos, k,
        [&]() { return launch_decimate_simple_ragged(log2decim, fcpos, in, in_stride, out, out_stride, max_raw, S, 0, 0, rows_dev, c->stream); },
        [&](DecimArgs &a, bool *mfma) -> int {
            if (frame_mode && !plan.mfma) return fail(SDRHIP_EINVAL, "internal: ragged frame mode needs the matrix-core launch");
            a.nsub_per_seg = plan.nsub; a.nseg = plan.grid;
            a.meta_rate = meta_rate;
            if (meta_w) memcpy(a.meta_w, meta_w, sizeof(a.meta_w));
            if (plan.mfma) {
                set_mf_args(a, plan.mf);
                a.mf_ring = plan.ring;
            }
            *mfma = plan.mfma;
            return SDRHIP_OK;
        },
        [&](const DecimArgs &a, bool pack16, bool mfma) {
            return mfma ? launch_decimate_mfma_ragged(log2decim, pack16, a, rows_dev, c->stream)
                        : launch_decimate_ragged(log2decim, fcpos, pack16, a, rows_dev, c->stream);
        });
}

int ragged_stage_in(sdrhip_ctx *c, PinnedBuf &pin, DevBuf &dev, const void *src, size_t in_stride, const size_t *n_in, int S, size_t esz,
                    size_t dstride, const void **out)
{
    int rc;
    size_t total = 0, max_n = 0;
    for (int s = 0; s < S; ++s) { total += n_in[s]; if (n_in[s] > max_n) max_n = n_in[s]; }
    const char *p = static_cast<const char *>(src);
    if ((size_t)S * dstride * esz <= SDRHIP_ZEROCOPY_MAX) {
        if ((rc = c->zin.reserve((size_t)S * dstride * esz + 16))) return rc;
        for (int s = 0; s < S; ++s)
            if (n_in[s]) memcpy(c->zin.as<char>() + (size_t)s * dstride * esz, p + (size_t)s * in_stride * esz, n_in[s] * esz);
        link_bytes(c, hipMemcpyHostToDevice, total * esz);
        *out = c->zin.p;
        return SDRHIP_OK;
    }
    if ((rc = pin.reserve((size_t)S * dstride * esz))) return rc;
    if ((rc = dev.reserve((size_t)S * dstride * esz + 16))) return rc;
    for (int s = 0; s < S; ++s)
// ... 225 lines not shown
```

sdrdaemon_amd/csrc/sdrhip_host.h:

```cpp
#pragma once
#include "../../include/sdrhip.h"
#include "dev_buffers.h"
#include "rx_stream_settings.h"
#include "sdrhip_internal.h"

#include <cstdint>
#include <cstring>
#include <atomic>
#include <map>
#include <mutex>
#include <string>
#include <utility>
#include <vector>

namespace sdrhip {

#define HIP_TRY(expr)                                                                                           \
    do {                                                                                                        \
        hipError_t e_ = (expr);                                                                                 \
        if (e_ != hipSuccess) return ::sdrhip::fail(SDRHIP_EDEVICE, "%s: %s", #expr, hipGetErrorString(e_));    \
    } while (0)

constexpr size_t SDRHIP_ZEROCOPY_MAX = (size_t)384 << 10;

inline bool aligned16(const void *p) { return (reinterpret_cast<uintptr_t>(p) & 15u) == 0; }
inline int check_mem(int mem)
{
    return mem == SDRHIP_MEM_HOST || mem == SDRHIP_MEM_DEVICE ? SDRHIP_OK : fail(SDRHIP_EINVAL, "mem must be SDRHIP_MEM_HOST or SDRHIP_MEM_DEVICE");
}

struct RxMeta {
    int first, count;
    unsigned frame_count0;
    unsigned w[6];
    uint64_t idx0;
    unsigned rate;
    const unsigned *tab;
};

int decimate_device(sdrhip_decimators *d, int log2decim, int fcpos, unsigned *sampleSize, const int16_t *in, size_t n_in,
                    size_t in_stride, int16_t *out, size_t out_stride, size_t *n_out, int frame_mode, int frame_blocks,
                    uint64_t frame_sample_base, const RxMeta *meta = nullptr, const Enc128Args *fuse = nullptr, bool *fused = nullptr,
                    bool coresident = false);
int ragged_prepare(sdrhip_decimators *d, int log2decim, int fcpos, const size_t *n_in, RaggedRow *rows, const RaggedRow **rows_dev,
                   RaggedPlan *plan, PinnedBuf *pin = nullptr);
int ragged_reserve(sdrhip_decimators *d, PinnedBuf *pin);
int decimate_ragged_device(sdrhip_decimators *d, int log2decim, int fcpos, unsigned *sampleSize, const int16_t *in, size_t in_stride,
                           int16_t *out, size_t out_stride, const RaggedRow *rows, const RaggedRow *rows_dev, const RaggedPlan &plan,
                           int frame_mode = 0, int frame_blocks = 0, const unsigned *meta_w = nullptr, unsigned meta_rate = 0);
int ragged_stage_in(sdrhip_ctx *c, PinnedBuf &pin, DevBuf &dev, const void *src, size_t in_stride, const size_t *n_in, int S, size_t esz,
                    size_t dstride, const void **out);
int ctx_stream2(sdrhip_ctx *c, hipStream_t *out);
bool decimate_mfma_applies(const sdrhip_decimators *d, int log2decim, int fcpos, size_t n_in);
struct InterpGather {
    const unsigned *map;
    const uint8_t *rx, *restored;
    int frames;
};
bool interpolate_gather_ok(const sdrhip_ctx *c, int log2interp);
struct InterpCount {
    const int *count;
    int stride, unit;
};
int interpolate_device(sdrhip_interpolators *p, int log2interp, const int16_t *in, size_t n_in, size_t in_stride, int16_t *out,
                       size_t out_stride, size_t *n_out, const InterpGather *gather = nullptr, const InterpCount *count = nullptr,
                       int out_fmt = IQF_S16,
                       const int *fmt_dev = nullptr);
int fecbuf_check_dgrams(const sdrhip_fecbuf *b, const uint8_t *dgrams, const size_t *n_dgrams, size_t dgram_stride_bytes, int mem, const char *who);
struct FecBufJoin {
    const unsigned *row_off;
    int (*admit)(void *arg, const size_t *n_frames);
    void *arg;
};
int fecbuf_collect(sdrhip_fecbuf *b, const uint8_t *dgrams, const size_t *n_dgrams, size_t dgram_stride_bytes, int mem, uint8_t *data_out,
                   size_t data_stride_bytes, uint8_t *block0_out, size_t max_frames, sdrhip_fecbuf_frame *info_out, size_t *n_frames,
                   const int **counts, const FecBufJoin *join = nullptr, const uint8_t *staged = nullptr);
int fecbuf_join_carry(sdrhip_fecbuf *b, unsigned **dev, std::vector<size_t> **host);
const FecBufState *fecbuf_committed_state(const sdrhip_fecbuf *b);
struct FecBufShadow {
    int head, count, recov, maxrow, dup;
    unsigned pres[4];
};
int fecbuf_shadow(sdrhip_fecbuf *b, std::vector<FecBufShadow> *out);
void fecbuf_shadow_run(FecBufShadow &h, const uint8_t *dg, size_t n, int res[4]);
void fecbuf_shadow_step(FecBufShadow &h, uint32_t hd, int res[4]);
int fecbuf_packed(sdrhip_fecbuf *b, const uint8_t *dg, const size_t *n_dgrams, const int *res, const std::vector<FecBufShadow> &next,
                  PinnedBuf &tab, uint8_t *data_out, size_t data_stride, uint8_t *block0_out, size_t max_frames, unsigned *mismatch,
                  bool *committed, const int **counts, const FecBufPub **pub, const FecBufJoin *join = nullptr);
struct FecBufBatch {
    int S;
    const uint8_t *dgrams;
    const size_t *n_dgrams;
    size_t stride;
    bool packed, inplace;
    size_t sum, nmax, bytes_in;
    size_t dev_bytes;
    const uint16_t *tags = nullptr;
    size_t n_total = 0;
    std::vector<size_t> counts;
    uint32_t *dest = nullptr;
};
int fecbuf_batch_check(FecBufBatch *in, int S, const uint8_t *dgrams, const size_t *n_dgrams, size_t dgram_stride_bytes, const char *who);
int fecbuf_batch_check_tagged(FecBufBatch *in, int S, const uint8_t *dgrams, const uint16_t *stream_of, size_t n_total, const char *who);
int fecbuf_batch_stage(FecBufBatch *in, PinnedBuf &arena, PinnedBuf &tab, std::vector<FecBufShadow> &sh, int *res);
int fecbuf_batch_upload(sdrhip_ctx *c, const FecBufBatch &in, PinnedBuf &arena, uint8_t *pk);
int fecbuf_tag_counts(int S, const uint8_t *dgrams, const uint16_t *stream_of, size_t n_total, const char *who, size_t *counts, size_t *sum,
                      size_t *nmax);
int fecbuf_batch_lost(const char *who, int rc);
constexpr size_t DG_REC = sizeof(sdrhip_fecbuf_frame);
static_assert(sizeof(sdrhip_fecbuf_frame) == sizeof(FecBufPub), "public record layout");
inline int reserve_settled(sdrhip_ctx *c, DevBuf &b, size_t n);
constexpr int DEC_STATS_SHADOW_MISMATCH = 1;
void fecbuf_set_async_busy(sdrhip_fecbuf *b, bool busy);
struct EncodeLin {
    const unsigned *lin;
    size_t stride;
    int cap, first, pending;
};
int enc128_min_rows(const sdrhip_ctx *c);
inline bool fec_encode_fuses_framing(const sdrhip_ctx *c, int nb_fec) { return nb_fec >= enc128_min_rows(c); }
int fec_encode_device(sdrhip_ctx *ctx, const uint8_t *frames, size_t frame_bytes, size_t nframes, int nb_fec, uint8_t *rec,
                      size_t rec_frame_bytes, const int32_t *frame_list_dev = nullptr, int ngroups = 0, const EncodeLin *lin = nullptr);
int fec_encode128_launch(sdrhip_ctx *ctx, const Enc128Args &k, hipStream_t on = nullptr);
struct DecodeSide {
    hipStream_t stream;
    DevBuf *plan, *idx;
    PinnedBuf *pin;
};
struct DecodeGather {
    unsigned *srcmap;
    uint8_t *restored;
    int rows;
};
bool fec_decode_gather_ok(const sdrhip_ctx *c);
int fec_decode_device(sdrhip_ctx *ctx, const uint8_t *rx, size_t rx_frame_bytes, const uint8_t *indices, size_t nframes,
                      uint8_t *payload_out, size_t payload_frame_bytes, uint8_t *block0_out, const DecodeSide *side = nullptr,
                      const DecodeGather *gather = nullptr, int max_rows = 0);
bool host_is_pinned(const void *p, size_t n);

typedef TableVersions StreamMask;
int stream_mask_upload(sdrhip_ctx *c, StreamMask &m, const uint8_t *mask, int S, const uint8_t **dev, int *n_set);
void decimators_reset_part(sdrhip_decimators *d, StreamResetArgs *a);
void decimators_reset_done(sdrhip_decimators *d, bool all);
void interpolators_reset_part(sdrhip_interpolators *p, StreamResetArgs *a);
void fecbuf_reset_part(sdrhip_fecbuf *b, StreamResetArgs *a);
void fecbuf_reset_done(sdrhip_fecbuf *b, const uint8_t *mask);
void fecbuf_fresh_state(FecBufState *x);
int stream_reset_launch(sdrhip_ctx *c, const StreamResetArgs &a);
int32_t *decimators_row(sdrhip_decimators *d, int s, int half);
int32_t *interpolators_row(sdrhip_interpolators *p, int s, int half);
bool decimators_stage0_int16(const sdrhip_decimators *d);
void decimators_clear_stage0_int16(sdrhip_decimators *d);
struct FecBufStreamRef {
    FecBufState *st[2];
    uint8_t *carry;
    size_t carry_half;
};
void fecbuf_stream_ref(sdrhip_fecbuf *b, int s, FecBufStreamRef *out);
void fecbuf_import_host(sdrhip_fecbuf *b, int s, const FecBufState &st, size_t carry);

}

#define SDRHIP_KCLASSES 5
namespace sdrhip {
struct CtxOptions {
    int decim_path = DECIM_PATH_AUTO;
    size_t mfma_span = 0;
    size_t mfma_min = (size_t)1 << 22;
    int interp_wave = 1;
    size_t interp_span = 0;
    int mfma_ring = 4;
    int rx_fused = 1;
    int rx_direct = 1;
    int rx_window = 0;
    int tx_overlap = 1;
    int enc_fft = 1;
    int enc_half = 0;
    int enc_bitslice = 1;
    int enc_min_rows = 1;
    int fec_stagger_mod = 0;
    int fec_stagger = 0;
    int tx_gather = 0;
    int dec_fused_plan = 1;
    int dec_syndrome = 1;
    int dec_strict = 0;
    int dec_max_rows = 128;
    int dec_auto = 0;
};
struct DecimPlanInfo {
    int path = 0;
    size_t span = 0, head = 0, tail_start = 0;
    int wps = 0, npieces = 0, nseg = 0;
};
}

struct sdrhip_ctx {
    std::recursive_mutex mtx;
    int device = 0;
    int n_cu = 256;
    sdrhip::CtxOptions opt;
    hipStream_t stream = nullptr;
    hipStream_t stream2 = nullptr;
    std::atomic<int> refs{0};
    std::atomic<bool> dying{false};
    sdrhip::DevBuf in, out, aux, aux3;
    uint8_t *gf_tab = nullptr;
    uint8_t *enc_matrix = nullptr;
    uint8_t *enc_leaves = nullptr;
    uint8_t *enc_fft = nullptr;
    unsigned *decim_dump = nullptr;
    unsigned *fused_roles = nullptr;
    unsigned fused_tag = 0;
    hipEvent_t ev0 = nullptr, ev1 = nullptr;
    uint8_t *gf_explog = nullptr;
    sdrhip::DevBuf dec_plan;
    unsigned *dec_stats = nullptr;
    sdrhip::PinnedBuf pin;
    sdrhip::PinnedBuf zin, zout;
    bool ktime_on = false;
    int ktime_stride = 1;
    int ktime_stride_cls[SDRHIP_KCLASSES] = {0, 0, 0, 0, 0};
    unsigned ktime_seen[SDRHIP_KCLASSES] = {0, 0, 0, 0, 0};
    std::vector<std::pair<hipEvent_t, hipEvent_t>> kev[SDRHIP_KCLASSES];
    uint64_t h2d_bytes = 0, d2h_bytes = 0;
};

namespace sdrhip {
struct CtxLock {
    std::lock_guard<std::recursive_mutex> g;
    explicit CtxLock(sdrhip_ctx *c) : g(c->mtx) {}
};
struct KTimer {
    sdrhip_ctx *c;
    int cls;
    hipEvent_t e1 = nullptr;
    hipStream_t st;
    KTimer(sdrhip_ctx *ctx, int kernel_class, hipStream_t on = nullptr) : c(ctx), cls(kernel_class), st(on ? on : ctx->stream)
    {
        if (!c->ktime_on) return;
        if (cls >= 0 && cls < SDRHIP_KCLASSES) {
            const int stride = c->ktime_stride_cls[cls] > 0 ? c->ktime_stride_cls[cls] : c->ktime_stride;
            if (stride > 1 && (c->ktime_seen[cls]++ % (unsigned)stride) != 0) return;
        }
        hipEvent_t e0 = nullptr;
        if (hipEventCreate(&e0) != hipSuccess) return;
        if (hipEventCreate(&e1) != hipSuccess) { (void)hipEventDestroy(e0); e1 = nullptr; return; }
        (void)hipEventRecord(e0, st);
        c->kev[cls].push_back(std::make_pair(e0, e1));
    }
    ~KTimer()
    {
        if (e1) (void)hipEventRecord(e1, st);
    }
};
inline int reserve_settled(sdrhip_ctx *c, DevBuf &b, size_t n)
{
    if (n > b.cap && b.p && hipStreamSynchronize(c->stream) != hipSuccess) return fail(SDRHIP_EDEVICE, "hipStreamSynchronize");
    return b.reserve(n);
}
inline void link_bytes(sdrhip_ctx *c, hipMemcpyKind kind, size_t bytes)
{
    if (kind == hipMemcpyHostToDevice) c->h2d_bytes += bytes;
    else if (kind == hipMemcpyDeviceToHost) c->d2h_bytes += bytes;
}
inline hipError_t link_copy(sdrhip_ctx *c, void *dst, const void *src, size_t bytes, hipMemcpyKind kind, hipStream_t stream)
{
    const hipError_t e = hipMemcpyAsync(dst, src, bytes, kind, stream);
    if (e == hipSuccess) link_bytes(c, kind, bytes);
    return e;
}
inline hipError_t link_copy2d(sdrhip_ctx *c, void *dst, size_t dpitch, const void *src, size_t spitch, size_t width, size_t height,
                              hipMemcpyKind kind, hipStream_t stream)
{
    const hipError_t e = hipMemcpy2DAsync(dst, dpitch, src, spitch, width, height, kind, stream);
    if (e == hipSuccess) link_bytes(c, kind, width * height);
    return e;
}
template <class F, class D> int stream_reset_bank(sdrhip_ctx *c, StreamMask &m, const uint8_t *mask, int S, F fill, D done)
{
    HIP_TRY(hipSetDevice(c->device));
    StreamResetArgs a;
    memset(&a, 0, sizeof(a));
    int n_set = 0;
    if (int rc = stream_mask_upload(c, m, mask, S, &a.mask, &n_set)) return rc;
    if (n_set == 0) return SDRHIP_OK;
    a.nstreams = S;
    fill(&a);
    if (int rc = stream_reset_launch(c, a)) return rc;
    done(n_set == S ? nullptr : mask);
    return SDRHIP_OK;
}
}
```

sdrdaemon_amd/csrc/sdrhip_internal.h:

```cpp
#pragma once
#include <hip/hip_runtime.h>
#include <stddef.h>
#include <stdint.h>

#include "decim_plan.h"
#include "interp_pick.h"
#include "interp_ragged_plan.h"
#include "rx_depart_order.h"
#include "rx_unpack_plan.h"

#ifndef SDRHIP_NT
#define SDRHIP_NT 1
#endif
#if SDRHIP_NT
#define SDRHIP_STREAM_LOAD(ptr) __builtin_nontemporal_load(ptr)
#else
#define SDRHIP_STREAM_LOAD(ptr) (*(ptr))
#endif

namespace sdrhip {

constexpr int DEC_STAGES = 6;
constexpr int DEC_HIST = 32;
constexpr int DEC_STATE_WORDS = DEC_STAGES * 4 * DEC_HIST;

constexpr int INT_STAGES = 6;
constexpr int INT_HIST = 32;
constexpr int INT_STATE_WORDS = INT_STAGES * 2 * INT_HIST;

struct DecimArgs {
    const int16_t *in;
    int16_t *out;
    size_t in_stride;
    size_t out_stride;
    size_t n_used;
    const int32_t *state_cur;
    int32_t *state_next;
    int nstreams;
    int nsub_per_seg;
    int nseg;
    int bias;
    int norm, trunk;
    int frame_mode;
    int frame_blocks;
    uint64_t frame_sample_base;
    int meta_first, meta_count;
    unsigned meta_frame_count0;
    unsigned meta_w[6];
    uint64_t meta_idx0;
    unsigned meta_rate;
    size_t mf_head, mf_span, mf_tail_start, mf_tail_seg;
    int mf_wps, mf_npieces;
    int mf_piece_wgs, mf_piece_early, mf_piece_share;
    unsigned *mf_dump;
    int mf_ring;
    int mf_prio;
    const unsigned *meta_tab;
};
template <class Args, class Meta> inline void set_meta_args(Args &a, const Meta &m)
{
    a.meta_first = m.first; a.meta_count = m.count; a.meta_frame_count0 = m.frame_count0;
    for (int i = 0; i < 6; ++i) a.meta_w[i] = m.w[i];
    a.meta_idx0 = m.idx0; a.meta_rate = m.rate; a.meta_tab = m.tab;
}

constexpr int STREAM_META_WORDS = 3;
#if defined(__HIPCC__) && __cplusplus >= 201703L
struct CrcBitTable { unsigned c[64]; };
constexpr CrcBitTable make_crc_bit_table()
{
    CrcBitTable T{};
    for (int k = 0; k < 64; ++k) {
        unsigned crc = 0u;
        for (int byte = 0; byte < 20; ++byte) {
            unsigned v = 0u;
            if (byte >= 12 && byte == 12 + k / 8) v = 1u << (k % 8);
            crc ^= v;
            for (int b = 0; b < 8; ++b) crc = (crc >> 1) ^ (0xEDB88320u & (0u - (crc & 1u)));
        }
        T.c[k] = crc;
    }
    return T;
}
__device__ const CrcBitTable CRC_BIT = make_crc_bit_table();

__device__ __forceinline__ void frame_meta_words(const unsigned (&base)[6], uint64_t idx0, unsigned rate, int fi, unsigned (&w)[6])
{
    unsigned sec = base[3], usec = base[4];
    if (rate) {
        const uint64_t idx = idx0 + (uint64_t)fi * 16129u;
        const uint64_t dus = idx * 1000000ull / rate;
        const uint64_t ds = dus / 1000000ull;
        usec += (unsigned)(dus - ds * 1000000ull);
        sec += (unsigned)ds;
        if (usec >= 1000000u) { usec -= 1000000u; sec += 1u; }
    }
    w[0] = base[0]; w[1] = base[1]; w[2] = base[2]; w[3] = sec; w[4] = usec;
    const int lane = (int)(threadIdx.x & 63u);
    const unsigned word = lane < 32 ? sec : usec;
    unsigned x = ((word >> (lane & 31)) & 1u) ? CRC_BIT.c[lane] : 0u;
#pragma unroll
    for (int m = 32; m >= 1; m >>= 1) x ^= (unsigned)__shfl_xor((int)x, m, 64);
    w[5] = base[5] ^ x;
}
__device__ __forceinline__ void frame_meta_words_thread(const unsigned (&base)[6], uint64_t idx0, unsigned rate, int fi, unsigned (&w)[6])
{
    unsigned sec = base[3], usec = base[4];
    if (rate) {
        const uint64_t idx = idx0 + (uint64_t)fi * 16129u;
        const uint64_t dus = idx * 1000000ull / rate;
        const uint64_t ds = dus / 1000000ull;
        usec += (unsigned)(dus - ds * 1000000ull);
        sec += (unsigned)ds;
        if (usec >= 1000000u) { usec -= 1000000u; sec += 1u; }
    }
    w[0] = base[0]; w[1] = base[1]; w[2] = base[2]; w[3] = sec; w[4] = usec;
    unsigned x = 0u;
#pragma unroll 8
    for (int k = 0; k < 32; ++k) {
        x ^= (0u - ((sec >> k) & 1u)) & CRC_BIT.c[k];
        x ^= (0u - ((usec >> k) & 1u)) & CRC_BIT.c[32 + k];
    }
    w[5] = base[5] ^ x;
}
template <bool ROW = false>
__device__ __forceinline__ void stream_meta_base(const unsigned (&shared)[6], unsigned shared_rate, const unsigned *p, int stream,
                                                 unsigned (&base)[6], unsigned &rate)
{
#pragma unroll
    for (int k = 0; k < 6; ++k) base[k] = shared[k];
    rate = shared_rate;
    if (ROW || p) {
        const unsigned *t = ROW ? p : p + (size_t)STREAM_META_WORDS * (size_t)__builtin_amdgcn_readfirstlane(stream);
        base[0] = t[0]; base[1] = t[1]; base[5] = t[2];
        if (ROW) base[2] = t[3];
        rate = t[1];
    }
}
#endif

hipError_t launch_decimate(int log2decim, int fcpos, bool pack16, const DecimArgs &a, hipStream_t stream);
hipError_t launch_decimate_mfma(int log2decim, bool pack16, const DecimArgs &a, hipStream_t stream);
struct Enc128Args;
constexpr int SDRHIP_FUSED_ROLE_WORDS = 4096 + 8;
hipError_t launch_rx_fused(int log2decim, bool pack16, const DecimArgs &a, const Enc128Args &e, unsigned *roles, unsigned tag, hipStream_t stream);

hipError_t launch_decimate_simple(int log2decim, int fcpos, const int16_t *in, size_t in_stride, int16_t *out,
                                  size_t out_stride, size_t n_in, int nstreams, int norm, int trunk,
                                  hipStream_t stream);

struct RaggedRow {
    uint64_t n_raw;
    uint64_t n_used;
    uint64_t n_dec;
    uint64_t out_off;
    uint64_t frame_sample_base;
    uint64_t meta_idx0;
    int seg0;
    int meta_first, meta_count;
    unsigned frame_count0;
    unsigned tv_sec, tv_usec;
    int mf_w0, mf_wps, mf_p0, mf_np;
    uint64_t mf_head, mf_tail_start;
    unsigned fc, rate, crc0;
    unsigned w2;
    unsigned shifts;
};
static_assert(sizeof(RaggedRow) == 128, "RaggedRow: one 128-byte row per stream");
hipError_t launch_decimate_mfma_ragged(int log2decim, bool pack16, const DecimArgs &a, const RaggedRow *rows, hipStream_t stream);
hipError_t launch_decimate_ragged(int log2decim, int fcpos, bool pack16, const DecimArgs &a, const RaggedRow *rows, hipStream_t stream);
constexpr int DECIM_TAP_SLOTS = 7;
struct DecimTapArgs {
    int16_t *out[DECIM_TAP_SLOTS];
    size_t stride[DECIM_TAP_SLOTS];
    int norm[DECIM_TAP_SLOTS], trunk[DECIM_TAP_SLOTS];
    unsigned mask;
};
hipError_t launch_decimate_taps(int log2decim, bool pack16, const DecimArgs &a, const DecimTapArgs &t, const RaggedRow *rows, hipStream_t stream);
hipError_t launch_decimate_simple_ragged(int log2decim, int fcpos, const int16_t *in, size_t in_stride, int16_t *out,
                                         size_t out_stride, size_t n_in, int nstreams, int norm, int trunk, const RaggedRow *rows,
                                         hipStream_t stream);

struct TestSourceParams {
    unsigned phase0;
    unsigned inc;
    int amp;
};
hipError_t launch_testsource(const int *table, const TestSourceParams *par, int16_t *out, size_t out_stride, size_t n, int nstreams,
                             hipStream_t stream);

struct FrameArgs {
    const unsigned *in;
    unsigned *out;
    size_t in_stride, out_stride;
    size_t n;
    size_t skip_from, skip_to;
    uint64_t frame_sample_base;
    int frame_blocks;
    int meta_first, meta_count;
    unsigned meta_frame_count0;
    unsigned meta_w[6];
    uint64_t meta_idx0;
    unsigned meta_rate;
    const unsigned *meta_tab;
};
hipError_t launch_frame_pack(const FrameArgs &a, int nstreams, hipStream_t stream);
hipError_t launch_frame_pack_ragged(const FrameArgs &a, const RaggedRow *rows, int nstreams, hipStream_t stream);
hipError_t launch_frame_meta_ragged(const FrameArgs &a, const RaggedRow *rows, int max_started, int nstreams, hipStream_t stream);

struct InterpArgs {
    const int16_t *in;
// ... 280 lines not shown
```

sdrdaemon_amd/csrc/sdrhip_rx.cpp:

```cpp
#include "sdrhip_pipes.h"

using namespace sdrhip;

static int rx_check_config(const sdrhip_rx_config *cfg);

extern "C" int sdrhip_rx_create(sdrhip_ctx *ctx, int nstreams, const sdrhip_rx_config *cfg, sdrhip_rx **out)
{
    if (!ctx || !cfg || !out || nstreams <= 0) return fail(SDRHIP_EINVAL, "rx_create: bad argument");
    {
        const int rcc = rx_check_config(cfg);
        if (rcc) return rcc;
    }
    sdrhip_rx *rx = new (std::nothrow) sdrhip_rx(ctx);
    if (!rx) return fail(SDRHIP_ENOMEM, "out of host memory");
    rx->nstreams = nstreams; rx->cfg = *cfg;
    rx->area.init((size_t)nstreams);
    rx->view.init((size_t)nstreams);
    rx->streams.init((size_t)nstreams);
    int rc = sdrhip_decimators_create(ctx, nstreams, cfg->hb_variant, &rx->dec);
    if (rc) { delete rx; return rc; }
    *out = rx;
    return SDRHIP_OK;
}

static int rx_check_config(const sdrhip_rx_config *cfg)
{
    if (cfg->log2decim < 0 || cfg->log2decim > 6) return fail(SDRHIP_EINVAL, "Invalid log2 decimation factor");
    if (cfg->fcpos < 0 || cfg->fcpos > 2) return fail(SDRHIP_EINVAL, "Invalid Fc position index");
    if (cfg->nb_fec < 0 || cfg->nb_fec > 128) return fail(SDRHIP_EINVAL, "nb_fec must be 0..128");
    if (cfg->sample_bits < 1 || cfg->sample_bits > 16) return fail(SDRHIP_EINVAL, "sample_bits must be 1..16");
    return SDRHIP_OK;
}

static int rx_settle(sdrhip_rx *rx)
{
    if (!rx->late.encode) return SDRHIP_OK;
    rx->late.encode = false;
    sdrhip_ctx *c = rx->ctx;
    if (c->opt.rx_fused != 3 || !rx->ev_framed) return fec_encode128_launch(c, rx->late.k);
    hipStream_t s2 = nullptr;
    int rc = ctx_stream2(c, &s2);
    if (rc) return rc;
    if ((rc = rx->ev_enc.ensure())) return rc;
    HIP_TRY(hipStreamWaitEvent(s2, rx->ev_framed, 0));
    if ((rc = fec_encode128_launch(c, rx->late.k, s2))) return rc;
    HIP_TRY(hipEventRecord(rx->ev_enc, s2));
    HIP_TRY(hipStreamWaitEvent(c->stream, rx->ev_enc, 0));
    return SDRHIP_OK;
}

extern "C" int sdrhip_rx_set_pipelined(sdrhip_rx *rx, int on)
{
    if (!rx) return fail(SDRHIP_EINVAL, "rx is NULL");
    sdrhip::CtxLock lock_(rx->ctx);
    if (!on && rx->late.have) return fail(SDRHIP_EINVAL, "rx_set_pipelined: sdrhip_rx_flush the waiting frames first");
    if (on && rx_refuse_uniform("rx_set_pipelined", nullptr, rx->streams.forces_ragged())) return SDRHIP_EINVAL;
    if (on && rx_dgrams_in_flight(rx)) return fail(SDRHIP_EINVAL, "rx_set_pipelined: asynchronous datagram batches are in flight: collect them first");
    if (on && !rx->area.aligned()) return fail(SDRHIP_EINVAL, "rx_set_pipelined: ragged calls left the streams at different frame positions");
    rx->pipelined = on ? 1 : 0;
    return SDRHIP_OK;
}

extern "C" int sdrhip_rx_set_input_format(sdrhip_rx *rx, int fmt)
{
    if (!rx) return fail(SDRHIP_EINVAL, "rx is NULL");
    sdrhip::CtxLock lock_(rx->ctx);
    if (fmt != SDRHIP_IQ_S16 && fmt != SDRHIP_IQ_U8 && fmt != SDRHIP_IQ_S8) return fail(SDRHIP_EINVAL, "rx_set_input_format: unknown format %d", fmt);
    if (rx->ring.busy()) return fail(SDRHIP_EINVAL, "rx_set_input_format: asynchronous batches are being filled or in flight: collect them first");
    if (rx->late.have) return fail(SDRHIP_EINVAL, "rx_set_input_format: frames of the previous call wait for delivery (pipelined mode): sdrhip_rx_flush them first");
    rx->in_fmt = fmt;
    return SDRHIP_OK;
}

static int rx_widen(sdrhip_rx *rx, const uint8_t *in, size_t in_stride, size_t n_in, size_t dstride, const int16_t **din)
{
    sdrhip_ctx *c = rx->ctx;
    int rc = rx->wide.reserve((size_t)rx->nstreams * dstride * 4 + 16);
    if (rc) return rc;
    hipError_t e;
    {
        KTimer kt(c, SDRHIP_K_CONVERT);
        e = launch_iq8_widen(rx->in_fmt, in, in_stride, rx->wide.as<int16_t>(), dstride, n_in, rx->nstreams, c->stream);
    }
    if (e != hipSuccess) return fail(SDRHIP_EDEVICE, "widen launch: %s", hipGetErrorString(e));
    *din = rx->wide.as<int16_t>();
    return SDRHIP_OK;
}

static int rx_release_old(sdrhip_rx *rx)
{
    if (rx->old_work.p && !(rx->late.have && rx->late.in_old)) {
        HIP_TRY(hipStreamSynchronize(rx->ctx->stream));
        rx->old_work.release();
    }
    return SDRHIP_OK;
}

static int rx_run_plan(sdrhip_rx *rx, const RxAreaPlan &p, DevBuf *fresh, size_t src_pitch, size_t dst_pitch, size_t bytes, const char *who)
{
    sdrhip_ctx *c = rx->ctx;
    const RxFrameArea &A = rx->area;
    const size_t S = A.streams(), dcap = fresh ? p.new_cap : A.cap();
    const uint8_t *src = rx->work.as<uint8_t>();
    uint8_t *dst = fresh ? fresh->as<uint8_t>() : rx->work.as<uint8_t>();
    bool together = true;
    for (size_t s = 0; s < S; ++s) together = together && p.to_slot0[s] && A.open(s) && A.slot(s) == A.slot(0);
    hipError_t e = hipSuccess;
    if (together)
        e = hipMemcpy2DAsync(dst, dcap * dst_pitch, src + A.slot(0) * src_pitch, A.cap() * src_pitch, bytes, S, hipMemcpyDeviceToDevice, c->stream);
    else
        for (size_t s = 0; s < S && e == hipSuccess; ++s)
            if (p.to_slot0[s] && A.open(s))
                e = hipMemcpyAsync(dst + s * dcap * dst_pitch, src + A.index(s) * src_pitch, bytes, hipMemcpyDeviceToDevice, c->stream);
    if (e == hipSuccess && fresh) e = hipStreamSynchronize(c->stream);
    if (e != hipSuccess) {
        if (fresh) { (void)hipStreamSynchronize(c->stream); fresh->release(); }
        return fail(SDRHIP_EDEVICE, "%s: moving the open frames: %s", who, hipGetErrorString(e));
    }
    if (fresh) {
        if (p.keep_old) { rx->old_work = std::move(rx->work); rx->late.in_old = true; }
        rx->work = std::move(*fresh);
        rx->view.clear();
    }
    rx->area.moved(p);
    return SDRHIP_OK;
}

static int rx_make_room(sdrhip_rx *rx, const size_t *done, bool pipelined, const char *who, bool grow_only = false)
{
    sdrhip_ctx *c = rx->ctx;
    const size_t wmul = c->opt.rx_window ? (size_t)c->opt.rx_window : pipelined ? 4 : 2;
    const RxAreaPlan p = rx->area.plan(done, rx->late.have && !rx->late.in_old ? rx->late.first : RX_NO_LATE, wmul);
    if (!p.new_cap && (grow_only || !p.moves())) return SDRHIP_OK;
    const size_t fb = rx_frame_bytes(rx);
    DevBuf fresh;
    if (p.new_cap)
        if (int rc = fresh.reserve(rx->area.streams() * p.new_cap * fb)) return rc;
    return rx_run_plan(rx, p, p.new_cap ? &fresh : nullptr, fb, fb, fb, who);
}

static int rx_repitch(sdrhip_rx *rx, size_t new_fb, const char *who)
{
    if (!rx->area.cap() || new_fb == rx_frame_bytes(rx)) return SDRHIP_OK;
    int rc;
    if ((rc = rx_settle(rx))) return rc;
    DevBuf fresh;
    if ((rc = fresh.reserve(rx->area.streams() * rx->area.cap() * new_fb))) return rc;
    if ((rc = rx_run_plan(rx, rx->area.replan(), &fresh, rx_frame_bytes(rx), new_fb, (size_t)SDRHIP_NB_ORIGINAL * SDRHIP_UDPSIZE, who))) return rc;
    rx->old_work.release();
    return SDRHIP_OK;
}

extern "C" int sdrhip_rx_reconfigure(sdrhip_rx *rx, const sdrhip_rx_config *cfg)
{
    if (!rx || !cfg) return fail(SDRHIP_EINVAL, "rx_reconfigure: NULL argument");
    sdrhip::CtxLock lock_(rx->ctx);
    int rc = rx_check_config(cfg);
    if (rc) return rc;
    if (cfg->hb_variant != rx->cfg.hb_variant) return fail(SDRHIP_EINVAL, "rx_reconfigure: hb_variant is fixed at creation");
    sdrhip_ctx *c = rx->ctx;
    HIP_TRY(hipSetDevice(c->device));
    const bool fec_changes = rx->streams.forces_ragged() != RX_SET_FEC && cfg->nb_fec != rx->cfg.nb_fec;
    if (fec_changes && rx->late.have)
        return fail(SDRHIP_EINVAL, "rx_reconfigure: frames of the previous call wait for delivery (pipelined mode): sdrhip_rx_flush them "
                                   "before changing fecblk (they carry the old frame size)");
    if (fec_changes && (rc = rx_repitch(rx, (size_t)(SDRHIP_NB_ORIGINAL + cfg->nb_fec) * SDRHIP_UDPSIZE, "rx_reconfigure"))) return rc;
    rx->cfg = *cfg;
    return SDRHIP_OK;
}

extern "C" void sdrhip_rx_destroy(sdrhip_rx *rx)
{
    if (!rx) return;
    sdrhip_ctx *c = rx->ctx;
    (void)hipSetDevice(c->device);
    (void)hipStreamSynchronize(c->stream);
    if (c->stream2) (void)hipStreamSynchronize(c->stream2);
    rx->ring.wait_all();
    sdrhip_decimators_destroy(rx->dec);
    sdrhip_fecbuf_destroy(rx->fb);
    delete rx;
}

extern "C" int sdrhip_rx_frames_view(const sdrhip_rx *rx, const uint8_t **base, size_t *stream_stride_bytes, size_t *n_frames)
{
    if (!rx || !base || !stream_stride_bytes || !n_frames) return fail(SDRHIP_EINVAL, "rx_frames_view: NULL argument");
    sdrhip::CtxLock lock_(rx->ctx);
    if (!rx->view.uniform()) return fail(SDRHIP_EINVAL, "rx_frames_view: the last call's windows differ between streams: use sdrhip_rx_frames_view_ragged");
    *base = rx->view.window(0, rx_frame_bytes(rx));
    *stream_stride_bytes = rx->view.stride();
    *n_frames = rx->view.frames(0);
    return SDRHIP_OK;
}

extern "C" int sdrhip_rx_frames_view_ragged(const sdrhip_rx *rx, const uint8_t **base, size_t *stream_stride_bytes, size_t *first_slot,
                                            size_t *n_frames)
{
    if (!rx || !base || !stream_stride_bytes || !first_slot || !n_frames) return fail(SDRHIP_EINVAL, "rx_frames_view_ragged: NULL argument");
    sdrhip::CtxLock lock_(rx->ctx);
    *base = rx->view.base();
    *stream_stride_bytes = rx->view.stride();
    for (size_t s = 0; s < (size_t)rx->nstreams; ++s) { first_slot[s] = rx->view.first(s); n_frames[s] = rx->view.frames(s); }
    return SDRHIP_OK;
}

extern "C" int sdrhip_rx_last_plan(const sdrhip_rx *rx, sdrhip_decim_plan *out)
{
    if (!rx) return fail(SDRHIP_EINVAL, "rx is NULL");
    return sdrhip_decimators_last_plan(rx->dec, out);
}

extern "C" size_t sdrhip_rx_max_frames(const sdrhip_rx *rx, size_t n_in)
{
    if (!rx) return 0;
    sdrhip::CtxLock lock_(rx->ctx);
    size_t now = 0;
    for (size_t s = 0; s < (size_t)rx->nstreams; ++s) {
        const size_t f = rx->area.advance(s, n_in >> rx->cfg.log2decim).done;
        if (f > now) now = f;
    }
    if (!rx->pipelined) return now;
    return rx->late.have && rx->late.frames > now ? rx->late.frames : now;
}

static int rx_deliver(sdrhip_rx *rx, const uint8_t *area, size_t first, size_t stride, size_t frames, size_t frame_bytes, uint8_t *frames_out,
                      size_t frame_stride_bytes, size_t *n_frames, int mem)
{
    sdrhip_ctx *c = rx->ctx;
    const int S = rx->nstreams;
    const uint8_t *base = area + first * frame_bytes;
    if (frames && frames_out) {
        if (S > 1 && frame_stride_bytes < frames * frame_bytes) return fail(SDRHIP_EINVAL, "rx_process: frame stride too small");
        HIP_TRY(link_copy2d(c, frames_out, S > 1 ? frame_stride_bytes : frames * frame_bytes, base, stride, frames * frame_bytes, S,
                            mem == SDRHIP_MEM_HOST ? hipMemcpyDeviceToHost : hipMemcpyDeviceToDevice, c->stream));
    } else if (frames && mem != SDRHIP_MEM_DEVICE) {
        return fail(SDRHIP_EINVAL, "rx_process: NULL frames_out");
    }
    rx->view.set(area, stride, (size_t)S, first, frames);
    if (n_frames) *n_frames = frames;
    return SDRHIP_OK;
}

extern "C" int sdrhip_rx_flush(sdrhip_rx *rx, uint8_t *frames_out, size_t frame_stride_bytes, size_t *n_frames, int mem)
{
    if (!rx) return fail(SDRHIP_EINVAL, "rx is NULL");
    sdrhip::CtxLock lock_(rx->ctx);
    if (n_frames) *n_frames = 0;
    if (int e = check_mem(mem)) return e;
    if (!rx->late.have) { rx->view.clear(); return SDRHIP_OK; }
    HIP_TRY(hipSetDevice(rx->ctx->device));
    int rc;
    if ((rc = rx_settle(rx))) return rc;
    if ((rc = rx_deliver(rx, rx->late.area, rx->late.first, rx->late.stride, rx->late.frames, rx->late.frame_bytes, frames_out, frame_stride_bytes, n_frames, mem))) return rc;
    rx->late.have = false;
    if (mem == SDRHIP_MEM_HOST) HIP_TRY(hipStreamSynchronize(rx->ctx->stream));
    return SDRHIP_OK;
}

static void rx_meta_base(const sdrhip_rx_config &cfg, unsigned ssd, unsigned w[6])
{
    rx_meta_record(cfg.center_frequency_khz, cfg.sample_rate, cfg.nb_fec, ssd, w);
}

static int rx_set_done(const RxSetResult &r, const char *who, const char *what, const char *range)
{
    if (r.kind == RxSetResult::RANGE) return fail(SDRHIP_EINVAL, "%s: %s[%zu] = %ld, must be %s", who, what, r.index, r.value, range);
    return r.kind == RxSetResult::NO_MEMORY ? fail(SDRHIP_ENOMEM, "out of host memory") : SDRHIP_OK;
}
static int rx_check_stream(const sdrhip_rx *rx, int stream, const char *who)
{
    return stream < 0 || stream >= rx->nstreams ? fail(SDRHIP_EINVAL, "%s: stream %d of %d", who, stream, rx->nstreams) : SDRHIP_OK;
}

extern "C" int sdrhip_rx_set_stream_meta(sdrhip_rx *rx, const uint32_t *center_frequency_khz, const uint32_t *sample_rate)
{
    if (!rx) return fail(SDRHIP_EINVAL, "rx is NULL");
    sdrhip::CtxLock lock_(rx->ctx);
    return rx_set_done(rx->streams.set_meta(center_frequency_khz, sample_rate), "rx_set_stream_meta", "", "");
}

extern "C" int sdrhip_rx_set_follow_meta(sdrhip_rx *rx, int on)
{
    if (!rx) return fail(SDRHIP_EINVAL, "rx is NULL");
    sdrhip::CtxLock lock_(rx->ctx);
    rx->follow_meta = on ? 1 : 0;
// ... 22 lines not shown
{
    if (!rx) return fail(SDRHIP_EINVAL, "rx is NULL");
    sdrhip::CtxLock lock_(rx->ctx);
    if (rx->pipelined || rx->late.have) return fail(SDRHIP_EINVAL, "rx_set_stream_fec: not available in pipelined mode");
    if (rx_batches_active(rx)) return fail(SDRHIP_EINVAL, "rx_set_stream_fec: asynchronous batches are being filled or in flight: collect them first");
    if (rx->ring.busy()) return fail(SDRHIP_EINVAL, "rx_set_stream_fec: a batch is lent (sdrhip_rx_collect_egress): sdrhip_rx_release_egress it first");
    if (int rc = rx_set_done(rx->streams.admit_fec(nb_fec), "rx_set_stream_fec", "nb_fec", "0..128")) return rc;
    HIP_TRY(hipSetDevice(rx->ctx->device));
    if (int rc = rx_repitch(rx, rx->streams.slot_blocks_of(nb_fec, rx_bank(rx)) * SDRHIP_UDPSIZE, "rx_set_stream_fec")) return rc;
    return rx_set_done(rx->streams.set_fec(nb_fec), "rx_set_stream_fec", "nb_fec", "0..128");
}

extern "C" int sdrhip_rx_get_stream_fec(const sdrhip_rx *rx, int stream, int *nb_fec, int *slot_blocks)
{
    if (!rx) return fail(SDRHIP_EINVAL, "rx is NULL");
    sdrhip::CtxLock lock_(rx->ctx);
    if (int e = rx_check_stream(rx, stream, "rx_get_stream_fec")) return e;
    if (nb_fec) *nb_fec = rx_fec_of(rx, (size_t)stream);
    if (slot_blocks) *slot_blocks = (int)(rx_frame_bytes(rx) / SDRHIP_UDPSIZE);
    return SDRHIP_OK;
}

extern "C" int sdrhip_rx_set_stream_bits(sdrhip_rx *rx, const unsigned *sample_bits)
{
    if (!rx) return fail(SDRHIP_EINVAL, "rx is NULL");
    sdrhip::CtxLock lock_(rx->ctx);
    if (rx->pipelined || rx->late.have) return fail(SDRHIP_EINVAL, "rx_set_stream_bits: not available in pipelined mode");
    return rx_set_done(rx->streams.set_bits(sample_bits), "rx_set_stream_bits", "sample_bits", "1..16");
}

extern "C" int sdrhip_rx_get_stream_bits(const sdrhip_rx *rx, int stream, unsigned *sample_bits, unsigned *frame_bits)
{
    if (!rx) return fail(SDRHIP_EINVAL, "rx is NULL");
    sdrhip::CtxLock lock_(rx->ctx);
    if (int e = rx_check_stream(rx, stream, "rx_get_stream_bits")) return e;
    const unsigned b = rx_bits_of(rx, (size_t)stream);
    if (sample_bits) *sample_bits = b;
    if (frame_bits) *frame_bits = decimated_sample_size((unsigned)rx->cfg.log2decim, b);
    return SDRHIP_OK;
}

extern "C" int sdrhip_rx_set_stream_format(sdrhip_rx *rx, const int *fmt)
{
    if (!rx) return fail(SDRHIP_EINVAL, "rx is NULL");
    sdrhip::CtxLock lock_(rx->ctx);
    if (rx->pipelined || rx->late.have) return fail(SDRHIP_EINVAL, "rx_set_stream_format: not available in pipelined mode");
    if (rx->ring.busy()) return fail(SDRHIP_EINVAL, "rx_set_stream_format: asynchronous batches are being filled or in flight: collect them first");
    return rx_set_done(rx->streams.set_format(fmt), "rx_set_stream_format", "fmt", "SDRHIP_IQ_S16, SDRHIP_IQ_U8 or SDRHIP_IQ_S8");
}

extern "C" int sdrhip_rx_get_stream_format(const sdrhip_rx *rx, int stream, int *fmt)
{
    if (!rx) return fail(SDRHIP_EINVAL, "rx is NULL");
    sdrhip::CtxLock lock_(rx->ctx);
    if (int e = rx_check_stream(rx, stream, "rx_get_stream_format")) return e;
    if (fmt) *fmt = rx->streams.format(rx->in_fmt, (size_t)stream);
    return SDRHIP_OK;
}

static int rx_stream_table(sdrhip_rx *rx, const unsigned **dev)
{
    *dev = nullptr;
    const RxStreamRecords *r = rx->streams.records(rx_bank(rx));
    if (!r) return SDRHIP_OK;
    if (rx->streams.changed()) {
        const void *tab = nullptr;
        if (int rc = rx->sm_tab.upload(rx->ctx->stream, r->words.data(), r->words.size() * sizeof(unsigned), &tab)) return rc;
        rx->streams.taken();
    }
    *dev = static_cast<const unsigned *>(rx->sm_tab.current());
    return SDRHIP_OK;
}

static int rx_stage_in(sdrhip_ctx *c, const void *src, size_t in_stride, size_t n_in, int S, size_t esz, size_t dstride, const void **out)
{
    int rc;
    if ((size_t)S * dstride * esz <= SDRHIP_ZEROCOPY_MAX) {
        if ((rc = c->zin.reserve((size_t)S * dstride * esz + 16))) return rc;
        for (int s = 0; s < S; ++s) memcpy(c->zin.as<char>() + (size_t)s * dstride * esz, static_cast<const char *>(src) + (size_t)s * in_stride * esz, n_in * esz);
        link_bytes(c, hipMemcpyHostToDevice, (size_t)S * n_in * esz);
        *out = c->zin.p;
    } else {
        if ((rc = c->in.reserve((size_t)S * dstride * esz + 16))) return rc;
        HIP_TRY(link_copy2d(c, c->in.p, dstride * esz, src, in_stride * esz, n_in * esz, S, hipMemcpyHostToDevice, c->stream));
        *out = c->in.p;
    }
    return SDRHIP_OK;
}

extern "C" int sdrhip_rx_process(sdrhip_rx *rx, const int16_t *iq_in, size_t n_in, size_t in_stride, uint32_t tv_sec, uint32_t tv_usec,
                                 uint8_t *frames_out, size_t frame_stride_bytes, size_t *n_frames, int mem)
{
    if (!rx) return fail(SDRHIP_EINVAL, "rx is NULL");
    sdrhip::CtxLock lock_(rx->ctx);
    if (n_frames) *n_frames = 0;
    if (int e = rx_refuse_uniform("rx_process", "sdrhip_rx_process_ragged", rx->streams.forces_ragged())) return e;
    if (rx_has_batches(rx, true)) return fail(SDRHIP_EINVAL, "rx_process: ragged batches are being filled or in flight: collect them first");
    if (rx_dgrams_in_flight(rx)) return fail(SDRHIP_EINVAL, "rx_process: asynchronous datagram batches are in flight: collect them first");
    if (n_in && !rx->area.aligned()) {
        const size_t S = (size_t)rx->nstreams;
        std::vector<size_t> cnt(S, n_in), nf(S, 0);
        std::vector<uint32_t> sec(S, tv_sec), usec(S, tv_usec);
        const int rc = rx_ragged(rx, iq_in, rx_counts(rx, cnt.data()), in_stride, sec.data(), usec.data(), frames_out, frame_stride_bytes, nf.data(), mem);
        if (rc) return rc;
        size_t most = 0;
        for (size_t s = 0; s < S; ++s) if (nf[s] > most) most = nf[s];
        if (n_frames) *n_frames = most;
        return SDRHIP_OK;
    }
    if (n_in == 0) {
        if (rx->pipelined && rx->late.have) return sdrhip_rx_flush(rx, frames_out, frame_stride_bytes, n_frames, mem);
        rx->view.clear();
        return SDRHIP_OK;
    }
    if (!iq_in) return fail(SDRHIP_EINVAL, "rx_process: NULL input");
    sdrhip_ctx *c = rx->ctx;
    rx->consumed = false;
    HIP_TRY(hipSetDevice(c->device));
    const int S = rx->nstreams, L = rx->cfg.log2decim, R = rx->cfg.nb_fec;
    const int FB = SDRHIP_NB_ORIGINAL + R;
    const size_t frame_bytes = (size_t)FB * SDRHIP_UDPSIZE;
    const size_t n_dec = n_in >> L;
    const uint64_t pending = rx->area.pending(0);
    const RxAdvance adv = rx->area.advance(0, n_dec);
    const size_t done = adv.done;
    if (S == 1) in_stride = n_in;
    const size_t deliver_now = rx->pipelined ? (rx->late.have ? rx->late.frames : 0) : done;
    const size_t deliver_fb = rx->pipelined && rx->late.have ? rx->late.frame_bytes : frame_bytes;
    if (deliver_now && !frames_out && mem != SDRHIP_MEM_DEVICE) return fail(SDRHIP_EINVAL, "rx_process: NULL frames_out");
    if (frames_out && S > 1 && deliver_now && frame_stride_bytes < deliver_now * deliver_fb) return fail(SDRHIP_EINVAL, "rx_process: frame stride too small");

    const int16_t *din = iq_in;
    size_t dstride = in_stride;
    int rc;
    const bool wide8 = rx->in_fmt != IQF_S16;
    const void *src = iq_in;
    if ((rc = check_mem(mem))) return rc;
    if (mem == SDRHIP_MEM_HOST) {
        dstride = wide8 ? (n_in + 7) & ~(size_t)7 : (n_in + 3) & ~(size_t)3;
        if ((rc = rx_stage_in(c, iq_in, in_stride, n_in, S, wide8 ? 2 : 4, dstride, &src))) return rc;
    } else if (!aligned16(iq_in) || (S > 1 && (in_stride & (wide8 ? 7 : 3)))) {
        return wide8 ? fail(SDRHIP_EALIGN, "rx_process: 8-bit device input must be 16-byte aligned, its stride a multiple of 8 samples")
                     : fail(SDRHIP_EALIGN, "rx_process: device input must be 16-byte aligned");
    }
    din = static_cast<const int16_t *>(src);
    if (wide8) {
        const size_t sstride = dstride;
        dstride = (n_in + 3) & ~(size_t)3;
        if ((rc = rx_widen(rx, static_cast<const uint8_t *>(src), sstride, n_in, dstride, &din))) return rc;
    }

    const std::vector<size_t> dones((size_t)S, done);
    if ((rc = rx_release_old(rx))) return rc;
    if ((rc = rx_make_room(rx, dones.data(), rx->pipelined != 0, "rx_process"))) return rc;
    const size_t cap = rx->area.cap(), slot0 = rx->area.slot(0);
    const size_t stream_bytes = cap * frame_bytes;
    uint8_t *work = rx->work.as<uint8_t>() + slot0 * frame_bytes;

    unsigned ss = rx->cfg.sample_bits;
    RxMeta meta;
    memset(&meta, 0, sizeof(meta));
    if (adv.started > 0) {
        rx_meta_base(rx->cfg, decimated_sample_size((unsigned)L, ss), meta.w);
        if ((rc = rx_stream_table(rx, &meta.tab))) return rc;
        meta.w[3] = tv_sec; meta.w[4] = tv_usec;
        meta.first = adv.first_new; meta.count = adv.started; meta.frame_count0 = adv.frame_count0;
        meta.idx0 = adv.idx0;
        meta.rate = rx->cfg.sample_rate;
    }

    size_t n_out = 0;
    EncodeLin elin;
    bool use_lin = false, pack_with_encoder = false;
    FrameArgs fa;
    memset(&fa, 0, sizeof(fa));
    const bool structured = R >= enc128_min_rows(c) && frame_bytes % 4 == 0;
    const bool filterless = L == 0 || (rx->cfg.fcpos != SDRHIP_FC_CEN && L <= 2);
    const Enc128Args *fuse = rx->late.encode && (c->opt.rx_fused == 1 || c->opt.rx_fused == 2) ? &rx->late.k : nullptr;
    const bool coresident = rx->late.encode && c->opt.rx_fused == 3 && rx->ev_framed;
    bool fused = false;
    const bool direct = c->opt.rx_direct && !rx->pipelined && stream_bytes < 0x3fffffffu;
    if (filterless || (!direct && decimate_mfma_applies(rx->dec, L, rx->cfg.fcpos, n_in))) {
        const size_t lstride = (n_dec + 3) & ~(size_t)3;
        if (rx->pipelined) rx->lin_sel ^= 1;
        DevBuf &lin = rx->lin[rx->lin_sel];
        if (lin.cap < (size_t)S * lstride * 4 + 16 && rx->late.encode) { if ((rc = rx_settle(rx))) return rc; fuse = nullptr; HIP_TRY(hipStreamSynchronize(c->stream)); }
        if ((rc = lin.reserve((size_t)S * lstride * 4 + 16))) return rc;
        rc = decimate_device(rx->dec, L, rx->cfg.fcpos, &ss, din, n_in, dstride, lin.as<int16_t>(), lstride, &n_out, 0, 0, 0, nullptr, fuse, &fused, coresident);
        if (rc) return rc;
        rx->consumed = true;
        if (fused) rx->late.encode = false;
        if (fec_encode_fuses_framing(c, R)) {
            const size_t first = pending ? 1 : 0;
            if (done > first && frame_bytes % 4 == 0) {
                elin.lin = lin.as<unsigned>(); elin.stride = lstride; elin.cap = (int)cap;
                elin.first = (int)first; elin.pending = (int)pending;
                use_lin = true;
            }
        }
        if (use_lin) {
            fa.skip_from = (size_t)elin.first * SDRHIP_SAMPLES_PER_FRAME - (size_t)elin.pending;
            fa.skip_to = done * SDRHIP_SAMPLES_PER_FRAME - (size_t)elin.pending;
        }
        fa.in = lin.as<unsigned>(); fa.out = reinterpret_cast<unsigned *>(work);
        fa.in_stride = lstride; fa.out_stride = stream_bytes / 4;
        fa.n = n_dec; fa.frame_sample_base = pending; fa.frame_blocks = FB;
        set_meta_args(fa, meta);
        pack_with_encoder = !rx->pipelined && c->opt.rx_fused && structured && R > 0 && use_lin;
        if (!pack_with_encoder) {
            hipError_t e = launch_frame_pack(fa, S, c->stream);
            if (e != hipSuccess) return fail(SDRHIP_EDEVICE, "frame pack launch: %s", hipGetErrorString(e));
        }
    } else {
        rc = decimate_device(rx->dec, L, rx->cfg.fcpos, &ss, din, n_in, dstride, reinterpret_cast<int16_t *>(work), stream_bytes / 4, &n_out, 1,
                             FB, pending, &meta);
        if (rc) return rc;
        rx->consumed = true;
    }
    if ((rc = rx_settle(rx))) return rc;

    bool encode_later = false;
    Enc128Args k;
    memset(&k, 0, sizeof(k));
    if (done && R > 0) {
        if (structured) {
            k.in = work; k.out = work + (size_t)SDRHIP_NB_ORIGINAL * SDRHIP_UDPSIZE; k.tab = c->gf_tab; k.leaf_tables = c->enc_leaves; k.fft_tables = c->enc_fft; k.use_fft = c->opt.enc_fft;
            k.bitslice = c->opt.enc_bitslice;
            k.in_frame_bytes = frame_bytes; k.out_frame_bytes = frame_bytes;
            k.rows = R; k.nframes = (int)((size_t)S * cap);
            k.nlist = (int)((size_t)S * done); k.gen_done = (int)done; k.gen_cap = (int)cap;
            if (use_lin) { k.lin = elin.lin; k.lin_stride = elin.stride; k.lin_cap = elin.cap; k.lin_first = elin.first; k.lin_pending = elin.pending; }
            if (rx->pipelined) {
                encode_later = true;
            } else if (pack_with_encoder) {
                set_meta_args(k, meta);
                if (elin.first == 1) { k.lin_straddle = 1; fa.skip_from = 0; }
                hipError_t e;
                {
                    KTimer kt(c, SDRHIP_K_FEC_ENCODE);
                    e = launch_gf_encode128_pack(k, fa, S, c->stream);
                }
                if (e != hipSuccess) return fail(SDRHIP_EDEVICE, "encode + frame pack launch: %s", hipGetErrorString(e));
            } else if ((rc = fec_encode128_launch(c, k))) return rc;
        } else {
            if (rx->flist_done != done || rx->flist_cap != cap) {
                HIP_TRY(hipStreamSynchronize(c->stream));
                rx->flist_host.clear();
                for (int s = 0; s < S; ++s)
                    for (size_t f = 0; f < done; ++f) rx->flist_host.push_back((int32_t)(s * cap + f));
                while (rx->flist_host.size() % GF_FRAMES_PER_GROUP) rx->flist_host.push_back(-1);
                if ((rc = rx->flist.reserve(rx->flist_host.size() * 4))) return rc;
                HIP_TRY(link_copy(c, rx->flist.p, rx->flist_host.data(), rx->flist_host.size() * 4, hipMemcpyHostToDevice, c->stream));
                rx->flist_done = done; rx->flist_cap = cap;
            }
            if ((rc = fec_encode_device(c, work, frame_bytes, (size_t)S * cap, R, work + (size_t)SDRHIP_NB_ORIGINAL * SDRHIP_UDPSIZE,
                                        frame_bytes, rx->flist.as<int32_t>(), (int)(rx->flist_host.size() / GF_FRAMES_PER_GROUP), nullptr)))
                return rc;
        }
    }
    if (rx->pipelined) {
        if (rx->late.have) {
            if ((rc = rx_deliver(rx, rx->late.area, rx->late.first, rx->late.stride, rx->late.frames, rx->late.frame_bytes, frames_out, frame_stride_bytes, n_frames, mem))) return rc;
        } else {
            rx->view.clear();
        }
        rx->late.have = done > 0;
        rx->late.encode = encode_later;
        if (encode_later && c->opt.rx_fused == 3) {
            if ((rc = rx->ev_framed.ensure())) return rc;
            HIP_TRY(hipEventRecord(rx->ev_framed, c->stream));
        }
        rx->late.k = k;
        rx->late.area = rx->work.as<uint8_t>(); rx->late.first = slot0; rx->late.in_old = false;
        rx->late.stride = stream_bytes; rx->late.frames = done; rx->late.frame_bytes = frame_bytes;
    } else {
        if ((rc = rx_deliver(rx, rx->work.as<uint8_t>(), slot0, stream_bytes, done, frame_bytes, frames_out, frame_stride_bytes, n_frames, mem))) return rc;
    }
    rx->area.commit(dones.data(), std::vector<uint64_t>((size_t)S, adv.rest).data());
    if (mem == SDRHIP_MEM_HOST) HIP_TRY(hipStreamSynchronize(c->stream));
    return SDRHIP_OK;
}

int sdrhip::rx_area_room(sdrhip_rx *rx, const size_t *done)
{
    return rx_make_room(rx, done ? done : std::vector<size_t>(rx->area.streams(), 0).data(), false, "rx_process_ragged", true);
}

static size_t rx_flist_entries(size_t sum_done) { return (sum_done / GF_FRAMES_PER_GROUP + 3) * GF_FRAMES_PER_GROUP; }
static int rx_encode_form(const sdrhip_ctx *c, int rows) { return rows < enc128_min_rows(c) ? 0 : rows <= 32 ? 1 : 2; }

int sdrhip::rx_ragged_room(sdrhip_rx *rx, const RxRaggedCounts &n, RxTabs *tabs)
{
    const int S = rx->nstreams, L = rx->cfg.log2decim;
    int rc;
    if ((rc = rx_area_room(rx, n.done.data()))) return rc;
    if ((rc = ragged_reserve(rx->dec, tabs ? &tabs->rows : nullptr))) return rc;
    const bool may_direct = rx->cfg.fcpos == SDRHIP_FC_CEN && L >= 2 && rx->ctx->opt.rx_direct;
    if (!may_direct && (rc = rx->lin[0].reserve((size_t)S * ((n.max_dec + 3) & ~(size_t)3) * 4 + 16))) return rc;
    if (n.sum_done && rx_fec_max(rx) > 0) {
        const size_t nl = rx_flist_entries(n.sum_done);
        if ((rc = (tabs ? tabs->flist : rx->r_flist_pin).reserve(nl * 4))) return rc;
        if ((rc = rx->r_flist.reserve(nl * 4))) return rc;
    }
    return SDRHIP_OK;
}

void sdrhip::rx_pack_rows(char *dst, const void *src, size_t pitch, const size_t *n_in, const int *fmts, int bank_fmt, size_t S)
{
    const char *rows = static_cast<const char *>(src), *packed = rows;
    for (size_t s = 0; s < S; ++s) {
        const size_t bytes = n_in[s] * unpackx_sample_bytes(fmts ? fmts[s] : bank_fmt);
        if (bytes) memcpy(dst, pitch ? rows + s * pitch : packed, bytes);
        dst += bytes;
        packed += bytes;
    }
}

int sdrhip::rx_unpack_launch(sdrhip_rx *rx, PinnedBuf &pin, DevBuf &dev, size_t tab_bytes, const int *fmts, const void *src, int16_t *out,
                             size_t dstride, unsigned grid)
{
    sdrhip_ctx *c = rx->ctx;
    const int S = rx->nstreams;
    HIP_TRY(hipMemcpyAsync(dev.p, pin.p, tab_bytes, hipMemcpyHostToDevice, c->stream));
    pin.mark(c->stream);
    const UnpackXRow *rows = dev.as<UnpackXRow>();
    const UnpackXSeg *segs = reinterpret_cast<const UnpackXSeg *>(rows + S + 1);
    hipError_t e;
    {
        KTimer kt(c, SDRHIP_K_CONVERT);
        e = fmts ? launch_unpack_mixed(src, out, dstride, rows, segs, S, grid, c->stream)
                 : launch_unpack_packed(rx->in_fmt, static_cast<const uint8_t *>(src), out, dstride, rows, segs, S, grid, c->stream);
    }
    if (e != hipSuccess) return fail(SDRHIP_EDEVICE, "unpack launch: %s", hipGetErrorString(e));
    return SDRHIP_OK;
}

static int rx_unpack_rows(sdrhip_rx *rx, const int16_t *iq_in, size_t in_stride, const size_t *n_in, const int *fmts, bool in_dev,
                          const int16_t **din, size_t *dstride)
{
    sdrhip_ctx *c = rx->ctx;
    const size_t S = (size_t)rx->nstreams;
    const UnpackXPlan m = unpackx_measure(n_in, 1, S, fmts);
    size_t max_in = 0;
    for (size_t s = 0; s < S; ++s) if (n_in[s] > max_in) max_in = n_in[s];
    const size_t rows_bytes = (S + 1) * sizeof(UnpackXRow), tab_bytes = rows_bytes + (size_t)m.nseg * sizeof(UnpackXSeg);
    const size_t ds = (max_in + 7) & ~(size_t)7;
    int rc;
    if ((rc = rx->f_tab_pin.reserve(tab_bytes))) return rc;
    if ((rc = reserve_settled(c, rx->f_tab, tab_bytes))) return rc;
    if ((rc = rx->wide.reserve(S * ds * 4 + 16))) return rc;
    const void *src = iq_in;
    if (!in_dev) {
        if ((rc = rx->f_pin.reserve((size_t)m.bytes))) return rc;
        if ((rc = reserve_settled(c, rx->f_pk, (size_t)m.bytes + 64))) return rc;
        rx_pack_rows(rx->f_pin.as<char>(), iq_in, in_stride * 4, n_in, fmts, 0, S);
        HIP_TRY(link_copy(c, rx->f_pk.p, rx->f_pin.p, (size_t)m.bytes, hipMemcpyHostToDevice, c->stream));
        rx->f_pin.mark(c->stream);
        src = rx->f_pk.p;
    }
    if (!unpackx_fill(n_in, 1, S, fmts, in_dev ? 2 * (uint64_t)in_stride : 0, rx->f_tab_pin.as<UnpackXRow>(),
                      reinterpret_cast<UnpackXSeg *>(rx->f_tab_pin.as<char>() + rows_bytes)).fits)
        return fail(SDRHIP_EINVAL, "rx_process_ragged: too many samples for one launch");
    if ((rc = rx_unpack_launch(rx, rx->f_tab_pin, rx->f_tab, tab_bytes, fmts, src, rx->wide.as<int16_t>(), ds, (unsigned)m.grid))) return rc;
    *din = rx->wide.as<int16_t>();
    *dstride = ds;
    return SDRHIP_OK;
}

int sdrhip::rx_ragged(sdrhip_rx *rx, const int16_t *iq_in, const RxRaggedCounts &n, size_t in_stride, const uint32_t *tv_sec, const uint32_t *tv_usec,
                      uint8_t *frames_out, size_t frame_stride_bytes, size_t *n_frames, int mem, bool batch, bool dev_rows, RxTabs *tabs,
                      const FecBufState *follow, const FecBufState *follow_bits)
{
    sdrhip_ctx *c = rx->ctx;
    const int S = rx->nstreams, L = rx->cfg.log2decim, R = rx_fec_max(rx);
    const size_t FB = (size_t)SDRHIP_NB_ORIGINAL + (size_t)R;
    const size_t frame_bytes = FB * SDRHIP_UDPSIZE;
    const bool mixed = rx_fec_mixed(rx);
    const size_t *n_in = n.n_in, max_in = n.max_in, max_dec = n.max_dec, max_done = n.max_done, sum_done = n.sum_done;
    const std::vector<size_t> &done = n.done;
    for (int s = 0; s < S; ++s) n_frames[s] = 0;
    if (int e = check_mem(mem)) return e;
    if (rx->pipelined) return fail(SDRHIP_EINVAL, "rx_process_ragged: not available in pipelined mode");
    if (!batch && rx_batches_active(rx)) return fail(SDRHIP_EINVAL, "rx_process_ragged: asynchronous batches are being filled or in flight: collect them first");
    if (S == 1) in_stride = max_in;
    if (S > 1 && in_stride < max_in) return fail(SDRHIP_EINVAL, "rx_process_ragged: in_stride smaller than the largest count");
    if (max_in && !iq_in) return fail(SDRHIP_EINVAL, "rx_process_ragged: NULL input");
    const int *fmts = !batch && !dev_rows ? rx->streams.formats() : nullptr;
    const bool wide8 = rx->in_fmt != IQF_S16 && !batch && !dev_rows && !fmts;
    const bool in_dev = mem == SDRHIP_MEM_DEVICE || dev_rows;
    if (fmts && !unpackx_measure(n_in, 1, (size_t)S, fmts).fits) return fail(SDRHIP_EINVAL, "rx_process_ragged: too many samples for one launch");
    if (max_in && in_dev && (!aligned16(iq_in) || (S > 1 && (in_stride & (wide8 ? 7 : 3)))))
        return fail(SDRHIP_EALIGN, "rx_process_ragged: device input must be 16-byte aligned, its stride a multiple of %d samples", wide8 ? 8 : 4);
    if (int e = rx_refuse_delivery("rx_process_ragged", n, frames_out, frame_stride_bytes, mem, false)) return e;
    HIP_TRY(hipSetDevice(c->device));
    rx->consumed = false;
    if (max_in == 0) {
        rx->view.clear();
        return SDRHIP_OK;
    }
    int rc;
    if ((rc = rx_release_old(rx))) return rc;
    if ((rc = rx_make_room(rx, done.data(), false, "rx_process_ragged"))) return rc;
    const RxFrameArea &A = rx->area;
    const size_t stream_bytes = A.cap() * frame_bytes;
    uint8_t *area = rx->work.as<uint8_t>();

    std::vector<unsigned> ss((size_t)S);
    for (int s = 0; s < S; ++s) ss[(size_t)s] = rx_bits_of(rx, (size_t)s);
    unsigned mw[6];
    rx_meta_base(rx->cfg, decimated_sample_size((unsigned)L, rx->cfg.sample_bits), mw);
    const RxStreamRecords *sw = rx->streams.records(rx_bank(rx));
    std::vector<RaggedRow> rows((size_t)S);
    memset(rows.data(), 0, rows.size() * sizeof(RaggedRow));
    for (int s = 0; s < S; ++s) {
        RaggedRow &r = rows[(size_t)s];
        const RxAdvance &a = n.adv[(size_t)s];
        r.out_off = A.slot((size_t)s) * frame_bytes / 4;
        r.frame_sample_base = A.pending((size_t)s);
        const unsigned *t = sw ? &sw->words[(size_t)s * STREAM_META_WORDS] : nullptr;
        r.fc = t ? t[0] : mw[0]; r.rate = t ? t[1] : mw[1];
        r.crc0 = t ? t[2] : mw[5];
        r.w2 = sw ? sw->w2[(size_t)s] : mw[2];
        r.shifts = sw ? sw->shifts[(size_t)s] : ragged_shift_word((unsigned)L, ss[(size_t)s]);
        if (a.started > 0 && (n_in[s] >> L)) {
            r.meta_first = a.first_new; r.meta_count = a.started;
            r.frame_count0 = a.frame_count0;
            r.meta_idx0 = a.idx0;
            r.tv_sec = tv_sec[s]; r.tv_usec = tv_usec[s];
        }
    }
    const RaggedRow *rdev = nullptr;
// ... 131 lines not shown
```

Baseline: 1.002 million.

## Write the open trailing frame directly to slot 0 to avoid ring wrap copies

When the frame area ring is about to wrap, the decimation kernel now writes the still-open last frame directly at slot 0 by shifting its output offsets (a new open-frame index and delta), instead of writing it at the ring tail and later copying it back with a device-to-device memcpy. This touches the host area planner, the commit logic, the scalar and MFMA output paths, and the buffer-resource base. It adds per-store index comparisons and extra offset arithmetic, and it only applies in the non-pipelined, direct, MFMA-admitted configuration. A counter for wrap copies is added.

```diff
diff --git a/sdrdaemon_amd/csrc/decim_body.h b/sdrdaemon_amd/csrc/decim_body.h
--- a/sdrdaemon_amd/csrc/decim_body.h
+++ b/sdrdaemon_amd/csrc/decim_body.h
@@ -59,7 +59,11 @@
     int norm, trunk;
     int frame_mode, frame_blocks;
     uint64_t frame_sample_base;
+    unsigned open_index;
+    size_t open_ddw;
 };
+
+__device__ __forceinline__ size_t frame_open_dw(const OutCtx &oc, uint64_t f) { return f == oc.open_index ? oc.open_ddw : (size_t)0; }
 
 __device__ __forceinline__ unsigned final_pack(int i, int q, int norm, int trunk)
 {
@@ -77,7 +81,7 @@
         uint64_t f = g / 16129u;
         unsigned w = (unsigned)(g - f * 16129u);
         unsigned b = w / 127u, i = w - b * 127u;
-        oc.out[((size_t)f * oc.frame_blocks + 1 + b) * 128u + 1 + i] = v;
+        oc.out[((size_t)f * oc.frame_blocks + 1 + b) * 128u + 1 + i + frame_open_dw(oc, f)] = v;
     }
 }
 
@@ -175,17 +179,17 @@
                 if (k0 + r < valid) oc.out[k + r] = o[r];
         } else {
             const uint64_t g = oc.frame_sample_base + k;
-            const uint64_t f = g / 16129u;
+            uint64_t f = g / 16129u;
             const unsigned w = (unsigned)(g - f * 16129u);
             unsigned b = w / 127u, i = w - b * 127u;
-            size_t dw = ((size_t)f * oc.frame_blocks + 1 + b) * 128u + 1 + i;
+            size_t dw = ((size_t)f * oc.frame_blocks + 1 + b) * 128u + 1 + i + frame_open_dw(oc, f);
 #pragma unroll
             for (int r = 0; r < R; ++r) {
                 if (k0 + r < valid) oc.out[dw] = o[r];
                 ++i; ++dw;
                 if (i == 127u) {
                     i = 0; ++b; dw += 1;
-                    if (b == 127u) { b = 0; dw += ((size_t)oc.frame_blocks - 127u) * 128u; }
+                    if (b == 127u) { b = 0; dw += ((size_t)oc.frame_blocks - 127u) * 128u + frame_open_dw(oc, ++f); }
                 }
             }
         }
@@ -295,7 +299,7 @@
     }
 }
 
-template <int L, int FC, bool PACK16, bool TAB = true, class TAPS = NoTaps>
+template <int L, int FC, bool PACK16, bool TAB = true, class TAPS = NoTaps, bool OPEN = false>
 __device__ __forceinline__ void decim_piece(const DecimArgs &a, int *lds, int stream, size_t seg_start, size_t seg_end, bool from_state,
                                             bool store_state, int meta_id, int meta_n, TAPS *taps = nullptr)
 {
@@ -315,6 +319,11 @@
     OutCtx oc;
     oc.norm = a.norm; oc.trunk = a.trunk;
     oc.frame_mode = a.frame_mode; oc.frame_blocks = a.frame_blocks; oc.frame_sample_base = a.frame_sample_base;
+    if constexpr (OPEN) {
+        oc.open_index = (unsigned)a.frame_open_index; oc.open_ddw = (size_t)0 - (size_t)((0u - a.frame_open_delta) >> 2);
+    } else {
+        oc.open_index = ~0u; oc.open_ddw = 0;
+    }
     oc.out = reinterpret_cast<unsigned *>(a.out) + (size_t)stream * a.out_stride;
     oc.out_pos = seg_start >> L;
     if constexpr (TAPS::ON) {
@@ -329,14 +338,14 @@
         for (int fi = meta_id + tid * meta_n; fi < a.meta_count; fi += NT * meta_n) {
             unsigned w[6];
             frame_meta_words_thread(base, a.meta_idx0, rate, fi, w);
-            unsigned *fr = oc.out + (size_t)(a.meta_first + fi) * a.frame_blocks * 128u;
+            unsigned *fr = oc.out + (size_t)(a.meta_first + fi) * a.frame_blocks * 128u + frame_open_dw(oc, (uint64_t)(a.meta_first + fi));
             fr[0] = (a.meta_frame_count0 + (unsigned)fi) & 0xffffu;
 #pragma unroll
             for (int k = 0; k < 6; ++k) fr[1 + k] = w[k];
         }
         if (tid < 128) {
             for (int fi = meta_id; fi < a.meta_count; fi += meta_n) {
-                unsigned *fr = oc.out + (size_t)(a.meta_first + fi) * a.frame_blocks * 128u;
+                unsigned *fr = oc.out + (size_t)(a.meta_first + fi) * a.frame_blocks * 128u + frame_open_dw(oc, (uint64_t)(a.meta_first + fi));
                 const unsigned fidx = (a.meta_frame_count0 + (unsigned)fi) & 0xffffu;
                 if (tid >= 7) fr[tid] = 0u;
                 if (tid >= 1) fr[(size_t)tid * 128] = fidx | ((unsigned)tid << 16);
diff --git a/sdrdaemon_amd/csrc/decim_mfma.hip b/sdrdaemon_amd/csrc/decim_mfma.hip
--- a/sdrdaemon_amd/csrc/decim_mfma.hip
+++ b/sdrdaemon_amd/csrc/decim_mfma.hip
@@ -349,8 +349,9 @@
     mf_wait_vm<0>();
 }
 
-template <int NS, int NG = 0, bool FR = false> __device__ __forceinline__ void mf_wave(const DecimArgs &a, int gw, unsigned lds_addr)
-{
+template <int NS, int NG = 0, bool FR = false, bool OPEN = false> __device__ __forceinline__ void mf_wave(const DecimArgs &a, int gw, unsigned lds_addr)
+{
+    static_assert(!OPEN || FR, "the open frame's place is a matter of the frame layout");
     if (a.mf_prio) __builtin_amdgcn_s_setprio(3);
     constexpr int L = NS;
     constexpr int P = mf_period<NS>();
@@ -400,13 +401,34 @@
         if constexpr (FR) {
             unsigned *obase = reinterpret_cast<unsigned *>(a.out) + (size_t)stream * a.out_stride;
             oc.rsrc = __builtin_amdgcn_make_buffer_rsrc(obase, 0, 0x3fffffff, 0x00020000);
+            unsigned open_off = 0u, open_gap = 0u;
+            constexpr bool EARLY = OPEN && mf_dma_applies(NS), LATE = OPEN && !mf_dma_applies(NS);
+            if constexpr (EARLY) {
+                if (a.frame_open_delta) {
+                    const unsigned fbytes = 512u * (unsigned)a.frame_blocks;
+                    const unsigned window = 0u - a.frame_open_delta - (unsigned)a.frame_open_index * fbytes;
+                    oc.rsrc = __builtin_amdgcn_make_buffer_rsrc(reinterpret_cast<char *>(obase) - window, 0, (unsigned)a.out_stride * 4u, 0x00020000);
+                    const unsigned long long thr = (unsigned long long)(unsigned)a.frame_open_index * 16129u - a.frame_sample_base;
+                    open_off = window + (first >= thr ? a.frame_open_delta : 0u);
+                    open_gap = first < thr && first + 16129u >= thr ? a.frame_open_delta : 0u;
+                }
+            }
             const unsigned long long g = a.frame_sample_base + first;
             const unsigned long long f = g / 16129u;
             const unsigned w = (unsigned)(g - f * 16129u);
             oc.b = w / 127u; oc.c = w - oc.b * 127u;
-            oc.off = 4u * (unsigned)(((size_t)f * (size_t)a.frame_blocks + 1u + oc.b) * 128u + 1u + oc.c + 2u * (unsigned)comp);
+            oc.off = 4u * (unsigned)(((size_t)f * (size_t)a.frame_blocks + 1u + oc.b) * 128u + 1u + oc.c + 2u * (unsigned)comp) + open_off;
             oc.t0 = 127u - 2u * (unsigned)comp; oc.t1 = 126u - 2u * (unsigned)comp;
-            oc.gap = 4u * ((unsigned)a.frame_blocks * 128u - 16255u);
+            oc.gap = 4u * ((unsigned)a.frame_blocks * 128u - 16255u) + open_gap;
+            if constexpr (LATE) {
+                if (a.frame_open_delta) {
+                    const unsigned fbytes = 512u * (unsigned)a.frame_blocks;
+                    const unsigned window = 0u - a.frame_open_delta - (unsigned)a.frame_open_index * fbytes;
+                    oc.rsrc = __builtin_amdgcn_make_buffer_rsrc(reinterpret_cast<char *>(obase) - window, 0, (unsigned)a.out_stride * 4u, 0x00020000);
+                    oc.off += window + (f == (unsigned)a.frame_open_index ? a.frame_open_delta : 0u);
+                    oc.gap += f + 1u == (unsigned)a.frame_open_index ? a.frame_open_delta : 0u;
+                }
+            }
             oc.p = nullptr;
         } else {
             unsigned *obase = reinterpret_cast<unsigned *>(a.out) + (size_t)stream * a.out_stride;
@@ -469,12 +491,12 @@
             if (lx >= nitems || (j < a.mf_piece_early && lx >= nearly)) break;
             const int stream = lx / a.mf_npieces, piece = lx - stream * a.mf_npieces;
             if (piece == 0) {
-                decim_piece<L, 2, PACK16>(a, lds, stream, 0, a.mf_head, true, false, piece, a.mf_npieces);
+                decim_piece<L, 2, PACK16, true, NoTaps, FR>(a, lds, stream, 0, a.mf_head, true, false, piece, a.mf_npieces);
             } else {
                 const size_t s0 = a.mf_tail_start + (size_t)(piece - 1) * a.mf_tail_seg;
                 size_t s1 = s0 + a.mf_tail_seg;
                 if (s1 > a.n_used || piece == a.mf_npieces - 1) s1 = a.n_used;
-                decim_piece<L, 2, PACK16>(a, lds, stream, s0, s1, false, piece == a.mf_npieces - 1, piece, a.mf_npieces);
+                decim_piece<L, 2, PACK16, true, NoTaps, FR>(a, lds, stream, s0, s1, false, piece == a.mf_npieces - 1, piece, a.mf_npieces);
             }
             __syncthreads();
         }
@@ -483,7 +505,7 @@
     const int gw = __builtin_amdgcn_readfirstlane(bx * 4 + (int)(threadIdx.x >> 6));
     if (gw >= a.nstreams * a.mf_wps) return;
     MF_STAMP(gw, 0);
-    mf_wave<L, NG, FR>(a, gw, (unsigned)(size_t)(__attribute__((address_space(3))) char *)lds);
+    mf_wave<L, NG, FR, FR>(a, gw, (unsigned)(size_t)(__attribute__((address_space(3))) char *)lds);
     MF_STAMP(gw, 7);
 }
 __device__ __forceinline__ int mf_ragged_find(const RaggedRow *rows, int nstreams, int x, bool waves)
diff --git a/sdrdaemon_amd/csrc/rx_frame_area.h b/sdrdaemon_amd/csrc/rx_frame_area.h
--- a/sdrdaemon_amd/csrc/rx_frame_area.h
+++ b/sdrdaemon_amd/csrc/rx_frame_area.h
@@ -20,6 +20,7 @@
     size_t new_cap = 0;
     bool keep_old = false;
     std::vector<uint8_t> to_slot0;
+    bool open_to_slot0 = false;
     bool moves() const
     {
         for (size_t s = 0; s < to_slot0.size(); ++s)
@@ -86,6 +87,14 @@
         }
         return p;
     }
+    bool open_in_place(RxAreaPlan *p, size_t done) const
+    {
+        if (p->new_cap || p->moves() || !aligned() || base_.empty()) return false;
+        const size_t base = base_[0];
+        if (done < 1 || base < 1 || base + done + 1 > cap_ || base + 2 * (done + 1) <= cap_) return false;
+        p->open_to_slot0 = true;
+        return true;
+    }
     RxAreaPlan replan() const
     {
         RxAreaPlan p;
@@ -99,10 +108,10 @@
         for (size_t s = 0; s < base_.size(); ++s)
             if (p.to_slot0[s]) base_[s] = 0;
     }
-    void commit(const size_t *done, const uint64_t *rest)
+    void commit(const size_t *done, const uint64_t *rest, bool open_to_slot0 = false)
     {
         for (size_t s = 0; s < base_.size(); ++s) {
-            base_[s] += done[s];
+            base_[s] = open_to_slot0 ? 0 : base_[s] + done[s];
             pending_[s] = rest[s];
             open_[s] = rest[s] > 0 ? 1 : 0;
             count_[s] = (uint16_t)(count_[s] + done[s]);
diff --git a/sdrdaemon_amd/csrc/sdrhip.cpp b/sdrdaemon_amd/csrc/sdrhip.cpp
--- a/sdrdaemon_amd/csrc/sdrhip.cpp
+++ b/sdrdaemon_amd/csrc/sdrhip.cpp
@@ -69,7 +69,7 @@
         if (hipGetDeviceProperties(&prop, device) == hipSuccess && prop.multiProcessorCount > 0) c->n_cu = prop.multiProcessorCount;
         static const char *const keys[][2] = {{"SDRHIP_DECIM_PATH", "decim_path"}, {"SDRHIP_MFMA_SPAN", "mfma_span"}, {"SDRHIP_MFMA_MIN", "mfma_min"},
                                               {"SDRHIP_INTERP_PATH", "interp_path"}, {"SDRHIP_INTERP_SPAN", "interp_span"}, {"SDRHIP_RX_FUSED", "rx_fused"}, {"SDRHIP_RX_DIRECT", "rx_direct"},
-                                              {"SDRHIP_DEC_PATH", "dec_path"}, {"SDRHIP_ENC_PATH", "enc_path"}, {"SDRHIP_ENC_MIN_ROWS", "enc_min_rows"}, {"SDRHIP_MFMA_RING", "mfma_ring"}, {"SDRHIP_TX_OVERLAP", "tx_overlap"}, {"SDRHIP_RX_WINDOW", "rx_window"}, {"SDRHIP_FEC_STAGGER", "fec_stagger"}, {"SDRHIP_FEC_STAGGER_MOD", "fec_stagger_mod"}, {"SDRHIP_DEC_PLAN", "dec_plan"}, {"SDRHIP_TX_GATHER", "tx_gather"}, {"SDRHIP_ENC_UNITS", "enc_units"}, {"SDRHIP_ENC_FORM", "enc_form"}};
+                                              {"SDRHIP_DEC_PATH", "dec_path"}, {"SDRHIP_ENC_PATH", "enc_path"}, {"SDRHIP_ENC_MIN_ROWS", "enc_min_rows"}, {"SDRHIP_MFMA_RING", "mfma_ring"}, {"SDRHIP_TX_OVERLAP", "tx_overlap"}, {"SDRHIP_RX_WINDOW", "rx_window"}, {"SDRHIP_RX_OPEN_IN_PLACE", "rx_open_in_place"}, {"SDRHIP_FEC_STAGGER", "fec_stagger"}, {"SDRHIP_FEC_STAGGER_MOD", "fec_stagger_mod"}, {"SDRHIP_DEC_PLAN", "dec_plan"}, {"SDRHIP_TX_GATHER", "tx_gather"}, {"SDRHIP_ENC_UNITS", "enc_units"}, {"SDRHIP_ENC_FORM", "enc_form"}};
         for (size_t i = 0; i < sizeof(keys) / sizeof(keys[0]); ++i)
             if (const char *v = getenv(keys[i][0])) (void)sdrhip_ctx_set_option(c, keys[i][1], v);
     }
@@ -161,6 +161,7 @@
     else if (k == "rx_fused" && v == "overlap") c->opt.rx_fused = 3;
     else if (k == "rx_direct" && isnum && num <= 1) c->opt.rx_direct = (int)num;
     else if (k == "rx_window" && isnum && num <= 8) c->opt.rx_window = (int)num;
+    else if (k == "rx_open_in_place" && isnum && num <= 1) c->opt.rx_open_in_place = (int)num;
     else if (k == "mfma_ring" && isnum && num >= 2 && num <= 4) c->opt.mfma_ring = (int)num;
     else if (k == "tx_overlap" && isnum && num <= 1) c->opt.tx_overlap = (int)num;
     else if (k == "fec_stagger" && isnum && num <= 64) c->opt.fec_stagger = (int)num;
@@ -201,6 +202,7 @@
     sdrhip::CtxLock lock_(c);
     if (std::string(key) == "h2d_bytes") { *value = c->h2d_bytes; return SDRHIP_OK; }
     if (std::string(key) == "d2h_bytes") { *value = c->d2h_bytes; return SDRHIP_OK; }
+    if (std::string(key) == "rx_wrap_copies") { *value = c->rx_wrap_copies; return SDRHIP_OK; }
     const bool shadow = std::string(key) == "fecbuf_shadow_mismatch";
     const bool deferred = std::string(key) == "dec_deferred";
     if (std::string(key) != "dec_rows_exceeded" && !shadow && !deferred) return fail(SDRHIP_EINVAL, "ctx_get_counter: unknown key: %s", key);
diff --git a/sdrdaemon_amd/csrc/sdrhip_decim.cpp b/sdrdaemon_amd/csrc/sdrhip_decim.cpp
--- a/sdrdaemon_amd/csrc/sdrhip_decim.cpp
+++ b/sdrdaemon_amd/csrc/sdrhip_decim.cpp
@@ -96,6 +96,11 @@
     a.mf_head = p.head; a.mf_span = p.span; a.mf_tail_start = p.tail_start; a.mf_tail_seg = p.tail_seg;
     a.mf_wps = p.wps; a.mf_npieces = p.npieces;
     a.mf_piece_wgs = p.piece_wgs; a.mf_piece_early = p.piece_early; a.mf_piece_share = p.piece_share;
+}
+
+bool mf_open_in_place_fits(int log2decim, const MfPlan &p, size_t out_stride)
+{
+    return (p.span >> log2decim) <= MF_OPEN_SPAN_MAX && out_stride * 4 <= MF_OPEN_AREA_MAX;
 }
 
 struct DecimCall {
@@ -155,7 +160,8 @@
 namespace sdrhip {
 int decimate_device(sdrhip_decimators *d, int log2decim, int fcpos, unsigned *sampleSize, const int16_t *in, size_t n_in,
                     size_t in_stride, int16_t *out, size_t out_stride, size_t *n_out, int frame_mode, int frame_blocks,
-                    uint64_t frame_sample_base, const RxMeta *meta, const Enc128Args *fuse, bool *fused, bool coresident)
+                    uint64_t frame_sample_base, const RxMeta *meta, const Enc128Args *fuse, bool *fused, bool coresident,
+                    const RxOpenFrame *open)
 {
     if (fused) *fused = false;
     sdrhip_ctx *c = d->ctx;
@@ -184,6 +190,11 @@
             *mfma = (!frame_mode || mfma_frames) && mfma_admitted(env.decim_path, env.mfma_min, log2decim, n_used * (size_t)S) &&
                     plan_decimate_mfma(log2decim, fcpos, n_used, S, env.mfma_span, c->n_cu, a.mf_ring, &p);
             if (*mfma) set_mf_args(a, p);
+            if (open && open->delta) {
+                if (!*mfma || fuse || !mf_open_in_place_fits(log2decim, p, out_stride))
+                    return fail(SDRHIP_EINVAL, "internal: the open frame cannot be written to slot 0 by this launch");
+                a.frame_open_index = open->index; a.frame_open_delta = open->delta;
+            }
             return SDRHIP_OK;
         },
         [&](const DecimArgs &a, bool pack16, bool mfma) -> hipError_t {
@@ -208,6 +219,16 @@
             if (fused) *fused = true;
             return e;
         });
+}
+
+bool decimate_open_in_place_ok(const sdrhip_decimators *d, int log2decim, int fcpos, size_t n_in, size_t out_stride)
+{
+    const CtxOptions &env = d->ctx->opt;
+    const size_t n_used = (n_in >> log2decim) << log2decim;
+    MfPlan p;
+    return env.rx_direct && out_stride * 4 < 0x3fffffffu && mfma_admitted(env.decim_path, env.mfma_min, log2decim, n_used * (size_t)d->nstreams) &&
+           plan_decimate_mfma(log2decim, fcpos, n_used, d->nstreams, env.mfma_span, d->ctx->n_cu, env.mfma_ring, &p) &&
+           mf_open_in_place_fits(log2decim, p, out_stride);
 }
 
 bool decimate_mfma_applies(const sdrhip_decimators *d, int log2decim, int fcpos, size_t n_in)
diff --git a/sdrdaemon_amd/csrc/sdrhip_host.h b/sdrdaemon_amd/csrc/sdrhip_host.h
--- a/sdrdaemon_amd/csrc/sdrhip_host.h
+++ b/sdrdaemon_amd/csrc/sdrhip_host.h
@@ -38,10 +38,17 @@
     const unsigned *tab;
 };
 
+struct RxOpenFrame {
+    int index;
+    unsigned delta;
+};
+
 int decimate_device(sdrhip_decimators *d, int log2decim, int fcpos, unsigned *sampleSize, const int16_t *in, size_t n_in,
                     size_t in_stride, int16_t *out, size_t out_stride, size_t *n_out, int frame_mode, int frame_blocks,
                     uint64_t frame_sample_base, const RxMeta *meta = nullptr, const Enc128Args *fuse = nullptr, bool *fused = nullptr,
-                    bool coresident = false);
+                    bool coresident = false,
+                    const RxOpenFrame *open = nullptr);
+bool decimate_open_in_place_ok(const sdrhip_decimators *d, int log2decim, int fcpos, size_t n_in, size_t out_stride);
 int ragged_prepare(sdrhip_decimators *d, int log2decim, int fcpos, const size_t *n_in, RaggedRow *rows, const RaggedRow **rows_dev,
                    RaggedPlan *plan, PinnedBuf *pin = nullptr);
 int ragged_reserve(sdrhip_decimators *d, PinnedBuf *pin);
@@ -172,6 +179,7 @@
     int mfma_ring = 4;
     int rx_fused = 1;
     int rx_direct = 1;
+    int rx_open_in_place = 1;
     int rx_window = 0;
     int tx_overlap = 1;
     int enc_fft = 1;
@@ -223,6 +231,7 @@
     unsigned ktime_seen[SDRHIP_KCLASSES] = {0, 0, 0, 0, 0};
     std::vector<std::pair<hipEvent_t, hipEvent_t>> kev[SDRHIP_KCLASSES];
     uint64_t h2d_bytes = 0, d2h_bytes = 0;
+    uint64_t rx_wrap_copies = 0;
 };
 
 namespace sdrhip {
diff --git a/sdrdaemon_amd/csrc/sdrhip_internal.h b/sdrdaemon_amd/csrc/sdrhip_internal.h
--- a/sdrdaemon_amd/csrc/sdrhip_internal.h
+++ b/sdrdaemon_amd/csrc/sdrhip_internal.h
@@ -56,7 +56,11 @@
     int mf_ring;
     int mf_prio;
     const unsigned *meta_tab;
-};
+    int frame_open_index;
+    unsigned frame_open_delta;
+};
+constexpr size_t MF_OPEN_SPAN_MAX = 126 * 127;
+constexpr size_t MF_OPEN_AREA_MAX = (size_t)1 << 29;
 template <class Args, class Meta> inline void set_meta_args(Args &a, const Meta &m)
 {
     a.meta_first = m.first; a.meta_count = m.count; a.meta_frame_count0 = m.frame_count0;
diff --git a/sdrdaemon_amd/csrc/sdrhip_rx.cpp b/sdrdaemon_amd/csrc/sdrhip_rx.cpp
--- a/sdrdaemon_amd/csrc/sdrhip_rx.cpp
+++ b/sdrdaemon_amd/csrc/sdrhip_rx.cpp
@@ -106,12 +106,15 @@
     bool together = true;
     for (size_t s = 0; s < S; ++s) together = together && p.to_slot0[s] && A.open(s) && A.slot(s) == A.slot(0);
     hipError_t e = hipSuccess;
-    if (together)
+    if (together) {
         e = hipMemcpy2DAsync(dst, dcap * dst_pitch, src + A.slot(0) * src_pitch, A.cap() * src_pitch, bytes, S, hipMemcpyDeviceToDevice, c->stream);
-    else
+        ++c->rx_wrap_copies;
+    } else
         for (size_t s = 0; s < S && e == hipSuccess; ++s)
-            if (p.to_slot0[s] && A.open(s))
+            if (p.to_slot0[s] && A.open(s)) {
                 e = hipMemcpyAsync(dst + s * dcap * dst_pitch, src + A.index(s) * src_pitch, bytes, hipMemcpyDeviceToDevice, c->stream);
+                ++c->rx_wrap_copies;
+            }
     if (e == hipSuccess && fresh) e = hipStreamSynchronize(c->stream);
     if (e != hipSuccess) {
         if (fresh) { (void)hipStreamSynchronize(c->stream); fresh->release(); }
@@ -126,11 +129,12 @@
     return SDRHIP_OK;
 }
 
-static int rx_make_room(sdrhip_rx *rx, const size_t *done, bool pipelined, const char *who, bool grow_only = false)
+static int rx_make_room(sdrhip_rx *rx, const size_t *done, bool pipelined, const char *who, bool grow_only = false, bool *open_to_slot0 = nullptr)
 {
     sdrhip_ctx *c = rx->ctx;
     const size_t wmul = c->opt.rx_window ? (size_t)c->opt.rx_window : pipelined ? 4 : 2;
-    const RxAreaPlan p = rx->area.plan(done, rx->late.have && !rx->late.in_old ? rx->late.first : RX_NO_LATE, wmul);
+    RxAreaPlan p = rx->area.plan(done, rx->late.have && !rx->late.in_old ? rx->late.first : RX_NO_LATE, wmul);
+    if (open_to_slot0) *open_to_slot0 = rx->area.open_in_place(&p, done[0]);
     if (!p.new_cap && (grow_only || !p.moves())) return SDRHIP_OK;
     const size_t fb = rx_frame_bytes(rx);
     DevBuf fresh;
@@ -459,9 +463,13 @@
 
     const std::vector<size_t> dones((size_t)S, done);
     if ((rc = rx_release_old(rx))) return rc;
-    if ((rc = rx_make_room(rx, dones.data(), rx->pipelined != 0, "rx_process"))) return rc;
+    bool open_to_slot0 = false;
+    const bool may_open = c->opt.rx_open_in_place && !rx->pipelined && !rx->late.have && !rx->ring.busy() && !rx->egress &&
+                          decimate_open_in_place_ok(rx->dec, L, rx->cfg.fcpos, n_in, rx->area.cap() * frame_bytes / 4);
+    if ((rc = rx_make_room(rx, dones.data(), rx->pipelined != 0, "rx_process", false, may_open ? &open_to_slot0 : nullptr))) return rc;
     const size_t cap = rx->area.cap(), slot0 = rx->area.slot(0);
     const size_t stream_bytes = cap * frame_bytes;
+    const RxOpenFrame open_frame = {(int)done, open_to_slot0 ? 0u - (unsigned)((slot0 + done) * frame_bytes) : 0u};
     uint8_t *work = rx->work.as<uint8_t>() + slot0 * frame_bytes;
 
     unsigned ss = rx->cfg.sample_bits;
@@ -488,6 +496,7 @@
     bool fused = false;
     const bool direct = c->opt.rx_direct && !rx->pipelined && stream_bytes < 0x3fffffffu;
     if (filterless || (!direct && decimate_mfma_applies(rx->dec, L, rx->cfg.fcpos, n_in))) {
+        if (open_to_slot0) return fail(SDRHIP_EINVAL, "internal: rx_process: the open frame's place was decided for the frame-layout launch");
         const size_t lstride = (n_dec + 3) & ~(size_t)3;
         if (rx->pipelined) rx->lin_sel ^= 1;
         DevBuf &lin = rx->lin[rx->lin_sel];
@@ -520,7 +529,7 @@
         }
     } else {
         rc = decimate_device(rx->dec, L, rx->cfg.fcpos, &ss, din, n_in, dstride, reinterpret_cast<int16_t *>(work), stream_bytes / 4, &n_out, 1,
-                             FB, pending, &meta);
+                             FB, pending, &meta, nullptr, nullptr, false, &open_frame);
         if (rc) return rc;
         rx->consumed = true;
     }
@@ -583,7 +592,7 @@
     } else {
         if ((rc = rx_deliver(rx, rx->work.as<uint8_t>(), slot0, stream_bytes, done, frame_bytes, frames_out, frame_stride_bytes, n_frames, mem))) return rc;
     }
-    rx->area.commit(dones.data(), std::vector<uint64_t>((size_t)S, adv.rest).data());
+    rx->area.commit(dones.data(), std::vector<uint64_t>((size_t)S, adv.rest).data(), open_to_slot0);
     if (mem == SDRHIP_MEM_HOST) HIP_TRY(hipStreamSynchronize(c->stream));
     return SDRHIP_OK;
 }
```

After: 1.009 million, median of 6. About the same (+0.7%).
